# flynn-nrg/izpi

Measured on AMD Instinct MI355X. Metric: Msamples/sec (pixels x spp) at 1024x1024/512spp, higher is better.
Workload: dtype f64

## Files before the change

include/izpi_gpu.h:

```cpp
#ifndef IZPI_GPU_H
#define IZPI_GPU_H
#include <stddef.h>
#include <stdint.h>
#include "izpi_types.h"

#ifdef __cplusplus
extern "C" {
#endif

typedef struct izpi_ctx izpi_ctx;

typedef struct izpi_scene_desc {
  uint32_t abi_version;
  uint32_t num_nodes;
  uint32_t num_prims;
  uint32_t num_tris, num_spheres, num_lights, num_materials, num_textures;
  uint32_t num_spd;
  uint32_t flags;
  uint64_t num_texels;
  const izpi_bvh4_node* nodes;
  const uint32_t* prim_ref;
  const double* tri_v0;
  const double* tri_v1;
  const double* tri_v2;
  const double* tri_e1;
  const double* tri_e2;
  const double* tri_normal;
  const double* tri_tangent;
  const double* tri_bitangent;
  const double* tri_uv;
  const double* tri_area;
  const uint32_t* tri_mat;
  const double* sph_center0;
  const double* sph_center1;
  const double* sph_time;
  const double* sph_radius;
  const uint32_t* sph_mat;
  const uint32_t* light_ref;
  const izpi_material* materials;
  const izpi_texture* textures;
  const double* texels;
  const double* spd_wavelengths;
  const double* spd_values;
  izpi_camera camera;
} izpi_scene_desc;

enum {
  IZPI_SCENE_QUANTIZED_BVH = 1
};

enum {
  IZPI_SAMPLER_NORMAL = 1,
  IZPI_SAMPLER_COLOUR = 2,
  IZPI_SAMPLER_WIREFRAME = 3,
  IZPI_SAMPLER_ALBEDO = 4,
  IZPI_SAMPLER_SPECTRAL = 5
};
enum {
  IZPI_OUT_CANVAS = 0,
  IZPI_OUT_PACKED = 1
};

typedef struct izpi_render_tuning {
  uint32_t slots;
  uint32_t chunk_units;
  uint32_t rec_dense;
  uint32_t pool_div;
  uint32_t trace_chunk;
  uint32_t refill_min;
  uint32_t prim_weight;
  uint32_t flags;
  uint64_t tail_paths;
  uint32_t peer_timeout_ms;
  uint32_t pad_tuning;
} izpi_render_tuning;
enum {
  IZPI_TUNE_NO_DIST = 1,
  IZPI_TUNE_GENERAL_TRACE = 2,
  IZPI_TUNE_NO_LEAF_SHORTCUT = 4,
  IZPI_TUNE_SCALAR_SLAB = 8,
  IZPI_TUNE_NO_TAIL = 16,
  IZPI_TUNE_PASS_LOG = 32,
  IZPI_TUNE_NO_LDS_BVH = 64,
  IZPI_TUNE_NO_RAY_LDS = 128,
  IZPI_TUNE_NO_PRIM_LDS = 256,
  IZPI_TUNE_NO_PLACE_PICK = 512,
  IZPI_TUNE_NO_QNODES = 1024,
  IZPI_TUNE_NO_SHADE_STAGE = 2048
};

typedef struct izpi_render_req {
  uint32_t width, height;
  uint32_t spp;
  uint32_t max_depth;
  uint32_t sampler;
  uint32_t out_layout;
  uint32_t num_tiles;
  uint32_t num_bg_spd;
  const uint32_t* tiles;
  const double* bg_spd_wavelengths;
  const double* bg_spd_values;
  double background[3];
  uint64_t seed;
  uint32_t post;
  uint32_t abi_version;
  double exposure;
  const izpi_render_tuning* tuning;
  uint32_t accumulation;
  uint32_t pad_req;
  double ink[3];
} izpi_render_req;

enum { IZPI_ACC_RECURSIVE = 0, IZPI_ACC_FORWARD = 1 };

enum { IZPI_POST_NONE = 0, IZPI_POST_SPECTRAL = 1,
       IZPI_POST_GAMMA_CLAMP = 2 };

enum { IZPI_FILTER_GAMMA = 1,
       IZPI_FILTER_CLAMP = 2   };
#define IZPI_MAX_FILTERS 8

typedef struct izpi_render_stats {
  uint64_t rays;
  uint64_t node_visits;
  uint64_t tri_tests;
  uint64_t sph_tests;
  uint64_t light_tri_tests;
  uint64_t light_sph_tests;
  uint64_t samples;
  double kernel_ms;
  double shade_ms;
  double total_ms;
  uint32_t launches;
  uint32_t pad;
  uint64_t node_steps, prim_steps, leaf_shortcuts;
  double tail_ms;
  uint64_t tail_node_visits, tail_tri_tests, tail_sph_tests;
  uint64_t parks;
  uint64_t workspace_bytes, scene_bytes;
  uint32_t slots, rec_dense, pool_blocks, chunk_spp;
  double alloc_ms;
} izpi_render_stats;

typedef struct izpi_hit {
  double t, u, v;
  double p[3];
  double normal[3];
  uint32_t prim_ref;
  uint32_t hit;
} izpi_hit;

int izpi_gpu_open(int device, izpi_ctx** out);
int izpi_gpu_close(izpi_ctx* ctx);
const char* izpi_gpu_last_error(izpi_ctx* ctx);

int izpi_gpu_upload_scene(izpi_ctx* ctx, const izpi_scene_desc* scene);

int izpi_gpu_render(izpi_ctx* ctx, const izpi_render_req* req, double* out_host, izpi_render_stats* stats);

int izpi_gpu_prepare(izpi_ctx* ctx, const izpi_render_req* req);

int izpi_gpu_render_device(izpi_ctx* ctx, const izpi_render_req* req, double* out_dev, izpi_render_stats* stats);

int izpi_gpu_unpack_tiles(izpi_ctx* ctx, const izpi_render_req* req, const double* packed_dev, double* canvas_dev);

int izpi_gpu_spectral_post(izpi_ctx* ctx, const double* xyz_dev, double* rgba_dev, uint32_t width, uint32_t height,
                           double exposure);

int izpi_gpu_postprocess(izpi_ctx* ctx, double* canvas_dev, uint32_t width, uint32_t height, const uint32_t* filters,
                         const double* params, uint32_t num_filters);

typedef struct izpi_denoise_params {
  uint32_t iterations;
  uint32_t flags;
  double sigma_colour, sigma_normal, sigma_albedo;
} izpi_denoise_params;
#define IZPI_DENOISE_MAX_ITERATIONS 8
#define IZPI_DENOISE_DEFAULT_ITERATIONS 5
#define IZPI_DENOISE_DEFAULT_SIGMA_COLOUR 1.0
#define IZPI_DENOISE_DEFAULT_SIGMA_NORMAL 0.5
#define IZPI_DENOISE_DEFAULT_SIGMA_ALBEDO 0.5
int izpi_gpu_denoise_device(izpi_ctx* ctx, const double* colour_dev, const double* normal_dev, const double* albedo_dev,
                            double* out_dev, uint32_t width, uint32_t height, const izpi_denoise_params* p,
                            double* device_ms);
int izpi_gpu_denoise(izpi_ctx* ctx, const double* colour, const double* normal, const double* albedo, double* out,
                     uint32_t width, uint32_t height, const izpi_denoise_params* p, double* device_ms);

enum { IZPI_BVH_LBVH = 0,
       IZPI_BVH_PLOC = 1,
       IZPI_BVH_SAH = 0x100 };
int izpi_gpu_build_bvh4(izpi_ctx* ctx, const double* boxes, uint32_t n, uint32_t leaf_max, uint32_t method,
                        izpi_bvh4_node* nodes, uint32_t max_nodes, uint32_t* num_nodes, uint32_t* order, double* build_ms);

typedef struct izpi_multi izpi_multi;
int izpi_gpu_multi_open(const int* devices, uint32_t num_devices, izpi_multi** out);
int izpi_gpu_multi_close(izpi_multi* m);
const char* izpi_gpu_multi_last_error(izpi_multi* m);
uint32_t izpi_gpu_multi_size(izpi_multi* m);
izpi_ctx* izpi_gpu_multi_context(izpi_multi* m, uint32_t i);
int izpi_gpu_multi_upload_scene(izpi_multi* m, const izpi_scene_desc* scene);
int izpi_gpu_multi_prepare(izpi_multi* m, const izpi_render_req* req);
int izpi_gpu_multi_render(izpi_multi* m, const izpi_render_req* req, double* out_host, izpi_render_stats* stats);

#define IZPI_COMM_ID_BYTES 128
int izpi_gpu_comm_id(uint8_t* id );
int izpi_gpu_comm_init(izpi_ctx* ctx, uint32_t nranks, uint32_t rank, const uint8_t* id );
int izpi_gpu_render_rank(izpi_ctx* ctx, const izpi_render_req* req, double* out_dev, izpi_render_stats* stats);

int izpi_gpu_progress(izpi_ctx* ctx, uint64_t* samples_done, uint64_t* samples_total);
int izpi_gpu_multi_progress(izpi_multi* m, uint64_t* samples_done, uint64_t* samples_total);

enum { IZPI_SNAP_CANVAS = 0, IZPI_SNAP_DISPLAY = 1 };
int izpi_gpu_progressive_begin(izpi_ctx* ctx, const izpi_render_req* req, uint32_t step_spp);
int izpi_gpu_progressive_step(izpi_ctx* ctx, uint32_t spp, izpi_render_stats* stats);
int izpi_gpu_progressive_snapshot(izpi_ctx* ctx, uint32_t form, double* out_host);
int izpi_gpu_progressive_snapshot_device(izpi_ctx* ctx, uint32_t form, double* out_dev);
int izpi_gpu_progressive_end(izpi_ctx* ctx);
int izpi_gpu_multi_progressive_begin(izpi_multi* m, const izpi_render_req* req, uint32_t step_spp);
int izpi_gpu_multi_progressive_step(izpi_multi* m, uint32_t spp, izpi_render_stats* stats);
int izpi_gpu_multi_progressive_snapshot(izpi_multi* m, uint32_t form, double* out_host);
int izpi_gpu_multi_progressive_end(izpi_multi* m);

enum { IZPI_PROG_NOISE = 1 };
enum { IZPI_SNAP_NOISE = 2 };
typedef struct izpi_noise_params {
  double threshold, floor, tolerated;
  uint32_t min_spp;
  uint32_t flags;
} izpi_noise_params;
#define IZPI_NOISE_DEFAULT_THRESHOLD 0.25
#define IZPI_NOISE_DEFAULT_FLOOR 0.01
#define IZPI_NOISE_DEFAULT_TOLERATED 0.05
#define IZPI_NOISE_DEFAULT_MIN_SPP 8
typedef struct izpi_noise_stats {
  uint64_t pixels, nonfinite, above;
  double max_error, sum_error, device_ms;
  uint32_t done, converged;
} izpi_noise_stats;
int izpi_gpu_progressive_begin_ex(izpi_ctx* ctx, const izpi_render_req* req, uint32_t step_spp, uint32_t flags);
int izpi_gpu_progressive_noise(izpi_ctx* ctx, const izpi_noise_params* p, izpi_noise_stats* out);
int izpi_gpu_progressive_converge(izpi_ctx* ctx, const izpi_noise_params* p, izpi_render_stats* stats,
// ... 17 lines not shown
```

izpi_amd/_native.py:

```python
import ctypes as C
from pathlib import Path

ROOT = Path(__file__).resolve().parents[1]
LIB_PATH = ROOT / "izpi_amd" / "_lib" / "libizpi_gpu.so"

c_double_p = C.POINTER(C.c_double)
c_uint32_p = C.POINTER(C.c_uint32)
c_float_p = C.POINTER(C.c_float)

COMM_ID_BYTES = 128
IZPI_OK, IZPI_ERR_INVALID, IZPI_ERR_HIP, IZPI_ERR_NO_SCENE, IZPI_ERR_UNSUPPORTED, IZPI_ERR_DEVICE, IZPI_ERR_PEER = range(7)
IZPI_ABI_VERSION = 4
ACC_RECURSIVE, ACC_FORWARD = 0, 1
SCENE_QUANTIZED_BVH = 1
PRIM_TRIANGLE, PRIM_SPHERE = 0, 1
TEX_CONSTANT, TEX_IMAGE, TEX_SPECTRAL_GAUSSIAN, TEX_SPECTRAL_TABULATED, TEX_SPECTRAL_IMAGE = 1, 3, 5, 7, 9
MAT_DIELECTRIC, MAT_DIFFUSE_LIGHT, MAT_ISOTROPIC, MAT_LAMBERT, MAT_METAL, MAT_PBR = 1, 2, 3, 4, 5, 6
MATF_BEER_LAMBERT = 1
SAMPLER_NORMAL, SAMPLER_COLOUR, SAMPLER_WIREFRAME, SAMPLER_ALBEDO, SAMPLER_SPECTRAL = 1, 2, 3, 4, 5
OUT_CANVAS, OUT_PACKED = 0, 1
POST_NONE, POST_SPECTRAL, POST_GAMMA_CLAMP = 0, 1, 2
SNAP_CANVAS, SNAP_DISPLAY, SNAP_NOISE = 0, 1, 2
PROG_NOISE = 1
NOISE_DEFAULT_THRESHOLD, NOISE_DEFAULT_FLOOR, NOISE_DEFAULT_TOLERATED, NOISE_DEFAULT_MIN_SPP = 0.25, 0.01, 0.05, 8
FILTER_GAMMA, FILTER_CLAMP = 1, 2
MAX_FILTERS = 8
HOST_SKIP_BVH = 1
BVH_LBVH, BVH_PLOC = 0, 1
BVH_SAH = 0x100
BVH_PLOC_SAH = BVH_PLOC | BVH_SAH
DISPLACE_PER_TRIANGLE, DISPLACE_MESH = 0, 1
DISPLACE_MAX_LEVELS = 16
DENOISE_MAX_ITERATIONS = 8
DENOISE_DEFAULT_ITERATIONS = 5
DENOISE_DEFAULT_SIGMA_COLOUR, DENOISE_DEFAULT_SIGMA_NORMAL, DENOISE_DEFAULT_SIGMA_ALBEDO = 1.0, 0.5, 0.5


def prim_ref(kind, idx):
    return (kind << 31) | idx


class BVH4Node(C.Structure):
    _fields_ = [("min_x", C.c_float * 4), ("min_y", C.c_float * 4), ("min_z", C.c_float * 4),
                ("max_x", C.c_float * 4), ("max_y", C.c_float * 4), ("max_z", C.c_float * 4),
                ("child", C.c_int32 * 4), ("prim_count", C.c_int32 * 4)]


class Texture(C.Structure):
    _fields_ = [("kind", C.c_uint32), ("width", C.c_uint32), ("height", C.c_uint32),
                ("spd_offset", C.c_uint32), ("spd_count", C.c_uint32), ("pad0", C.c_uint32),
                ("texel_offset", C.c_uint64), ("value", C.c_double * 3),
                ("peak", C.c_double), ("center", C.c_double), ("width_nm", C.c_double)]


class Material(C.Structure):
    _fields_ = [("kind", C.c_uint32), ("albedo_tex", C.c_int32), ("spectral_tex", C.c_int32),
                ("normal_tex", C.c_int32), ("roughness_tex", C.c_int32), ("metalness_tex", C.c_int32),
                ("absorb_tex", C.c_int32), ("flags", C.c_uint32), ("ref_idx", C.c_double),
                ("fuzz", C.c_double), ("rgb", C.c_double * 3), ("pad1", C.c_double)]


class Camera(C.Structure):
    _fields_ = [("origin", C.c_double * 3), ("lower_left", C.c_double * 3), ("horizontal", C.c_double * 3),
                ("vertical", C.c_double * 3), ("u", C.c_double * 3), ("v", C.c_double * 3),
                ("lens_radius", C.c_double), ("time0", C.c_double), ("time1", C.c_double), ("exposure", C.c_double)]


class SceneDesc(C.Structure):
    _fields_ = [("abi_version", C.c_uint32), ("num_nodes", C.c_uint32), ("num_prims", C.c_uint32),
                ("num_tris", C.c_uint32), ("num_spheres", C.c_uint32), ("num_lights", C.c_uint32),
                ("num_materials", C.c_uint32), ("num_textures", C.c_uint32), ("num_spd", C.c_uint32),
                ("flags", C.c_uint32), ("num_texels", C.c_uint64),
                ("nodes", C.POINTER(BVH4Node)), ("prim_ref", c_uint32_p),
                ("tri_v0", c_double_p), ("tri_v1", c_double_p), ("tri_v2", c_double_p),
                ("tri_e1", c_double_p), ("tri_e2", c_double_p), ("tri_normal", c_double_p),
                ("tri_tangent", c_double_p), ("tri_bitangent", c_double_p), ("tri_uv", c_double_p),
                ("tri_area", c_double_p), ("tri_mat", c_uint32_p),
                ("sph_center0", c_double_p), ("sph_center1", c_double_p), ("sph_time", c_double_p),
                ("sph_radius", c_double_p), ("sph_mat", c_uint32_p),
                ("light_ref", c_uint32_p), ("materials", C.POINTER(Material)), ("textures", C.POINTER(Texture)),
                ("texels", c_double_p), ("spd_wavelengths", c_double_p), ("spd_values", c_double_p),
                ("camera", Camera)]


class RenderTuning(C.Structure):
    _fields_ = [("slots", C.c_uint32), ("chunk_units", C.c_uint32), ("rec_dense", C.c_uint32),
                ("pool_div", C.c_uint32), ("trace_chunk", C.c_uint32), ("refill_min", C.c_uint32),
                ("prim_weight", C.c_uint32), ("flags", C.c_uint32), ("tail_paths", C.c_uint64),
                ("peer_timeout_ms", C.c_uint32), ("pad_tuning", C.c_uint32)]


TUNE_NO_DIST, TUNE_GENERAL_TRACE, TUNE_NO_LEAF_SHORTCUT, TUNE_SCALAR_SLAB, TUNE_NO_TAIL, TUNE_PASS_LOG = 1, 2, 4, 8, 16, 32
TUNE_NO_LDS_BVH = 64
TUNE_NO_RAY_LDS = 128
TUNE_NO_PRIM_LDS = 256
TUNE_NO_QNODES = 1024
TUNE_NO_SHADE_STAGE = 2048


def tuning(**kw):
    t = RenderTuning()
    for k, v in kw.items():
        if k == "flags" and not isinstance(v, int):
            v = sum(v)
        setattr(t, k, v)
    return t


class RenderReq(C.Structure):
    _fields_ = [("width", C.c_uint32), ("height", C.c_uint32), ("spp", C.c_uint32), ("max_depth", C.c_uint32),
                ("sampler", C.c_uint32), ("out_layout", C.c_uint32), ("num_tiles", C.c_uint32),
                ("num_bg_spd", C.c_uint32), ("tiles", c_uint32_p), ("bg_spd_wavelengths", c_double_p),
                ("bg_spd_values", c_double_p), ("background", C.c_double * 3), ("seed", C.c_uint64),
                ("post", C.c_uint32), ("abi_version", C.c_uint32), ("exposure", C.c_double),
                ("tuning", C.POINTER(RenderTuning)), ("accumulation", C.c_uint32), ("pad_req", C.c_uint32),
                ("ink", C.c_double * 3)]


class RenderStats(C.Structure):
    _fields_ = [("rays", C.c_uint64), ("node_visits", C.c_uint64), ("tri_tests", C.c_uint64),
                ("sph_tests", C.c_uint64), ("light_tri_tests", C.c_uint64), ("light_sph_tests", C.c_uint64),
                ("samples", C.c_uint64), ("kernel_ms", C.c_double), ("shade_ms", C.c_double),
                ("total_ms", C.c_double), ("launches", C.c_uint32), ("pad", C.c_uint32),
                ("node_steps", C.c_uint64), ("prim_steps", C.c_uint64), ("leaf_shortcuts", C.c_uint64),
                ("tail_ms", C.c_double), ("tail_node_visits", C.c_uint64), ("tail_tri_tests", C.c_uint64),
                ("tail_sph_tests", C.c_uint64), ("parks", C.c_uint64), ("workspace_bytes", C.c_uint64),
                ("scene_bytes", C.c_uint64), ("slots", C.c_uint32), ("rec_dense", C.c_uint32),
                ("pool_blocks", C.c_uint32), ("chunk_spp", C.c_uint32), ("alloc_ms", C.c_double)]

    def as_dict(self):
        return {k: getattr(self, k) for k, _ in self._fields_ if k != "pad"}


class DenoiseParams(C.Structure):
    _fields_ = [("iterations", C.c_uint32), ("flags", C.c_uint32), ("sigma_colour", C.c_double),
                ("sigma_normal", C.c_double), ("sigma_albedo", C.c_double)]


def denoise_params(iterations=DENOISE_DEFAULT_ITERATIONS, sigma_colour=DENOISE_DEFAULT_SIGMA_COLOUR,
                   sigma_normal=DENOISE_DEFAULT_SIGMA_NORMAL, sigma_albedo=DENOISE_DEFAULT_SIGMA_ALBEDO):
    return DenoiseParams(int(iterations), 0, float(sigma_colour), float(sigma_normal), float(sigma_albedo))


class NoiseParams(C.Structure):
    _fields_ = [("threshold", C.c_double), ("floor", C.c_double), ("tolerated", C.c_double),
                ("min_spp", C.c_uint32), ("flags", C.c_uint32)]


def noise_params(threshold=NOISE_DEFAULT_THRESHOLD, floor=NOISE_DEFAULT_FLOOR, tolerated=NOISE_DEFAULT_TOLERATED,
                 min_spp=NOISE_DEFAULT_MIN_SPP):
    return NoiseParams(float(threshold), float(floor), float(tolerated), int(min_spp), 0)


class NoiseStats(C.Structure):
    _fields_ = [("pixels", C.c_uint64), ("nonfinite", C.c_uint64), ("above", C.c_uint64),
                ("max_error", C.c_double), ("sum_error", C.c_double), ("device_ms", C.c_double),
                ("done", C.c_uint32), ("converged", C.c_uint32)]

    def as_dict(self):
        return {k: getattr(self, k) for k, _ in self._fields_}


class Hit(C.Structure):
    _fields_ = [("t", C.c_double), ("u", C.c_double), ("v", C.c_double), ("p", C.c_double * 3),
                ("normal", C.c_double * 3), ("prim_ref", C.c_uint32), ("hit", C.c_uint32)]


class TriIn(C.Structure):
    _fields_ = [("v0", C.c_double * 3), ("v1", C.c_double * 3), ("v2", C.c_double * 3),
                ("uv", C.c_double * 6), ("material", C.c_uint32), ("pad", C.c_uint32)]


class SphereIn(C.Structure):
    _fields_ = [("center", C.c_double * 3), ("radius", C.c_double), ("material", C.c_uint32), ("pad", C.c_uint32)]


class CameraIn(C.Structure):
    _fields_ = [("look_from", C.c_double * 3), ("look_at", C.c_double * 3), ("vup", C.c_double * 3),
                ("vfov", C.c_double), ("aspect", C.c_double), ("aperture", C.c_double), ("focus_dist", C.c_double),
                ("time0", C.c_double), ("time1", C.c_double), ("exposure", C.c_double)]


class SceneInput(C.Structure):
    _fields_ = [("num_tris", C.c_uint32), ("num_spheres", C.c_uint32), ("num_materials", C.c_uint32),
                ("num_textures", C.c_uint32), ("num_spd", C.c_uint32), ("pad0", C.c_uint32),
                ("num_texels", C.c_uint64), ("tris", C.c_void_p), ("spheres", C.c_void_p),
                ("materials", C.POINTER(Material)), ("textures", C.POINTER(Texture)), ("texels", c_double_p),
                ("spd_wavelengths", c_double_p), ("spd_values", c_double_p), ("camera", CameraIn),
                ("aspect_override", C.c_double), ("bvh_seed", C.c_uint64)]


COLOUR_RGB, COLOUR_SPECTRAL = 1, 2
OBJ_IGNORE_NORMALS, OBJ_IGNORE_MATERIALS, OBJ_IGNORE_TEXTURES = 1, 2, 4
OBJ_FACE_POLYGON = 1


class ProtoInfo(C.Structure):
    _fields_ = [("colour_representation", C.c_uint32), ("stream_triangles", C.c_uint32),
                ("total_triangles", C.c_uint64), ("num_triangles", C.c_uint32), ("num_streamed_triangles", C.c_uint32),
                ("num_spheres", C.c_uint32), ("num_materials", C.c_uint32), ("num_image_textures", C.c_uint32),
                ("num_displacement_maps", C.c_uint32), ("num_background", C.c_uint32), ("pad", C.c_uint32),
                ("name", C.c_char_p), ("version", C.c_char_p), ("warnings", C.c_char_p)]


class ObjInfo(C.Structure):
    _fields_ = [("has_normals", C.c_uint32), ("has_uv", C.c_uint32), ("ignore_materials", C.c_uint32),
                ("ignore_normals", C.c_uint32), ("ignore_textures", C.c_uint32), ("num_groups", C.c_uint32),
                ("num_materials", C.c_uint32), ("pad", C.c_uint32), ("num_vertices", C.c_uint64),
                ("num_normals", C.c_uint64), ("num_uvs", C.c_uint64), ("centre", C.c_double * 3),
                ("object_name", C.c_char_p)]


class ObjGroup(C.Structure):
    _fields_ = [("name", C.c_char_p), ("material", C.c_char_p), ("face_type", C.c_uint32), ("is_null", C.c_uint32),
                ("num_faces", C.c_uint64), ("num_face_vertices", C.c_uint64)]


class ObjMaterial(C.Structure):
    _fields_ = [("name", C.c_char_p), ("kd", C.c_double * 3), ("ka", C.c_double * 3), ("ks", C.c_double * 3),
                ("num_kd", C.c_uint32), ("num_ka", C.c_uint32), ("num_ks", C.c_uint32), ("pad", C.c_uint32),
                ("ns", C.c_double), ("ni", C.c_double), ("d", C.c_double), ("sharpness", C.c_int64),
                ("illum", C.c_int64)]


ABI_STRUCTS = [BVH4Node, Texture, Material, Camera, SceneDesc, RenderReq, RenderStats, Hit, TriIn, SphereIn, CameraIn,
               SceneInput, ProtoInfo, ObjInfo, ObjGroup, ObjMaterial, RenderTuning, DenoiseParams, NoiseParams, NoiseStats]

EXPORTS = [
    "izpi_gpu_open", "izpi_gpu_close", "izpi_gpu_prepare", "izpi_gpu_multi_prepare", "izpi_gpu_last_error", "izpi_gpu_upload_scene", "izpi_gpu_render",
    "izpi_gpu_render_device", "izpi_gpu_unpack_tiles", "izpi_gpu_output_bytes", "izpi_gpu_trace",
    "izpi_gpu_ray_aabb4", "izpi_gpu_gomath", "izpi_gpu_spectral_post", "izpi_gpu_postprocess",
    "izpi_gpu_build_bvh4", "izpi_gpu_multi_open", "izpi_gpu_multi_close", "izpi_gpu_multi_last_error",
    "izpi_gpu_multi_size", "izpi_gpu_multi_context", "izpi_gpu_multi_upload_scene", "izpi_gpu_multi_render",
    "izpi_gpu_comm_id", "izpi_gpu_comm_init", "izpi_gpu_render_rank", "izpi_gpu_debug_fault", "izpi_gpu_debug_realloc", "izpi_gpu_progress", "izpi_gpu_multi_progress", "izpi_host_build_scene_ex", "izpi_host_scene_prim_boxes", "izpi_host_scene_set_bvh", "izpi_host_scene_set_flags",
    "izpi_host_build_scene", "izpi_host_scene_desc", "izpi_host_scene_stack_bound", "izpi_host_scene_build_ms",
    "izpi_host_scene_free", "izpi_host_last_error", "izpi_host_tiles", "izpi_host_share_units", "izpi_host_share_tiles", "izpi_host_share_block", "izpi_host_assemble_shares", "izpi_host_bvh_leaf_max", "izpi_host_gomath", "izpi_abi_struct_size",
    "izpi_scene_parse_text", "izpi_scene_parse_binary", "izpi_scene_serialize", "izpi_scene_info", "izpi_scene_image_file",
    "izpi_scene_set_image", "izpi_scene_add_triangles", "izpi_scene_background", "izpi_scene_to_input",
    "izpi_scene_material_name", "izpi_scene_free", "izpi_light_source", "izpi_light_source_name",
    "izpi_obj_parse", "izpi_obj_info_get", "izpi_obj_copy_vertices", "izpi_obj_group_get", "izpi_obj_copy_faces",
    "izpi_obj_material_get", "izpi_obj_translate", "izpi_obj_scale", "izpi_obj_rotate",
    "izpi_obj_group_to_triangles", "izpi_obj_free",
    "izpi_gpu_displace", "izpi_host_displace", "izpi_scene_displacement_file", "izpi_scene_set_displacement_map",
    "izpi_scene_set_displacer",
    "izpi_gpu_progressive_begin", "izpi_gpu_progressive_step", "izpi_gpu_progressive_snapshot",
    "izpi_gpu_progressive_snapshot_device", "izpi_gpu_progressive_end",
    "izpi_gpu_multi_progressive_begin", "izpi_gpu_multi_progressive_step", "izpi_gpu_multi_progressive_snapshot",
    "izpi_gpu_multi_progressive_end",
    "izpi_gpu_denoise_device", "izpi_gpu_denoise", "izpi_host_denoise",
    "izpi_gpu_progressive_begin_ex", "izpi_gpu_progressive_noise", "izpi_gpu_progressive_converge",
# ... 144 lines not shown
```

izpi_amd/csrc/izpi_dev.h:

```cpp
#pragma once
#include <hip/hip_runtime.h>
#include <stdint.h>
#include "../../include/izpi_gpu.h"
#include "gomath.h"
#include "scene_records.h"

#define IZPI_DEV __device__ __forceinline__

namespace izd {

struct DevScene {
  const GInner* inner;
  const GInnerQ* innerq;
  const GLeaf* leaves;
  const GPrim* prims;
  const GShade* shade;
  const GTriTex* tritex;
  const GLight* lights;
  const izpi_material* materials;
  const izpi_texture* textures;
  const double4* mat_const;
  const MatTex* mat_tex;
  const double* texels;
  const double* spd_wl;
  const double* spd_val;
  int32_t root;
  uint32_t num_lights;
  uint32_t nan_free_bounds;
  uint32_t leaf_shortcut;
  uint32_t tri_only;
  uint32_t no_pathlen;
  uint32_t num_inner;
  uint32_t num_prims;
  izpi_camera cam;
  uint32_t lds_bytes;
  uint32_t time_free;
  uint32_t quantized;
#ifdef IZPI_SHADOW
  const GInner* sh_inner;
  const GLeaf* sh_leaves;
  const GPrim* sh_prims;
#endif
};

struct RenderParams {
  uint32_t width, height, spp, max_depth;
  uint32_t chunk_spp;
  uint32_t s0;
  uint32_t num_pixels;
  uint32_t tile_w, tile_h;
  uint32_t total_units;
  uint32_t lanes;
  uint32_t num_bg_spd;
  const uint32_t* tiles;
  const double* bg_wl;
  const double* bg_val;
  double background[3];
  uint64_t seed;
  double* out;
  double* recs;
  uint32_t* head;
  unsigned long long* counters;
  uint32_t* error;
};

struct Lcg {
  uint32_t s;
  IZPI_DEV double next() {
    s = 1664525u * s + 1013904223u;
    return (double)s / 4294967296.0;
  }
};
IZPI_DEV uint64_t splitmix64(uint64_t x) {
  uint64_t z = x + 0x9E3779B97F4A7C15ull;
  z = (z ^ (z >> 30)) * 0xBF58476D1CE4E5B9ull;
  z = (z ^ (z >> 27)) * 0x94D049BB133111EBull;
  return z ^ (z >> 31);
}
#define IZPI_CAMERA_STREAM_SALT 0xD6E8FEB86659FD93ull

IZPI_DEV int64_t go_int(double x) {
  if (x != x || x >= 9223372036854775808.0 || x < -9223372036854775808.0) return INT64_MIN;
  return (int64_t)x;
}

struct V3 { double x, y, z; };
IZPI_DEV V3 mk(double x, double y, double z) { V3 r; r.x = x; r.y = y; r.z = z; return r; }
IZPI_DEV V3 ld3(const double* p) { return mk(p[0], p[1], p[2]); }
IZPI_DEV V3 add(V3 a, V3 b) { return mk(a.x + b.x, a.y + b.y, a.z + b.z); }
IZPI_DEV V3 sub(V3 a, V3 b) { return mk(a.x - b.x, a.y - b.y, a.z - b.z); }
IZPI_DEV V3 mul(V3 a, V3 b) { return mk(a.x * b.x, a.y * b.y, a.z * b.z); }
IZPI_DEV V3 smul(V3 a, double t) { return mk(a.x * t, a.y * t, a.z * t); }
IZPI_DEV bool sdiv_plain(double x) {
  return ((uint32_t)(__double2hiint(x) >> 20) & 0x7FFu) - (1023u - 300u) <= 600u;
}
IZPI_DEV V3 sdiv(V3 a, double t) {
  const int px = (int)sdiv_plain(a.x) | (int)(a.x == 0.0), py = (int)sdiv_plain(a.y) | (int)(a.y == 0.0),
            pz = (int)sdiv_plain(a.z) | (int)(a.z == 0.0);
  const bool plain = ((int)sdiv_plain(t) & px & py & pz) != 0;
  if (plain) {
    double r = __builtin_amdgcn_rcp(t);
    double e = __builtin_fma(-t, r, 1.0);
    r = __builtin_fma(r, e, r);
    e = __builtin_fma(-t, r, 1.0);
    r = __builtin_fma(r, e, r);
    auto q1 = [&](double n) {
      const double q = n * r;
      const double res = __builtin_fma(-t, q, n);
      return __builtin_amdgcn_div_fixup(__builtin_amdgcn_div_fmas(res, r, q, false), t, n);
    };
    return mk(q1(a.x), q1(a.y), q1(a.z));
  }
  return mk(a.x / t, a.y / t, a.z / t);
}
IZPI_DEV double dot(V3 a, V3 b) { return (a.x * b.x) + (a.y * b.y) + (a.z * b.z); }
IZPI_DEV V3 cross(V3 a, V3 b) { return mk((a.y * b.z) - (a.z * b.y), -((a.x * b.z) - (a.z * b.x)), (a.x * b.y) - (a.y * b.x)); }
IZPI_DEV double sqlen(V3 a) { return (a.x * a.x) + (a.y * a.y) + (a.z * a.z); }
IZPI_DEV double length(V3 a) { return gm::sqrt(sqlen(a)); }
IZPI_DEV V3 unit(V3 a) { return sdiv(a, length(a)); }
IZPI_DEV V3 lerp(V3 a, V3 b, double t) {
  return mk((1 - t) * a.x + t * b.x, (1 - t) * a.y + t * b.y, (1 - t) * a.z + t * b.z);
}
IZPI_DEV bool bad(double x) { return x != x || gm::is_inf(x, 0); }
IZPI_DEV V3 denan(V3 v) { return mk(bad(v.x) ? 0.0 : v.x, bad(v.y) ? 0.0 : v.y, bad(v.z) ? 0.0 : v.z); }

struct Onb {
  V3 u, v, w;
  IZPI_DEV void build(V3 n) {
    w = unit(n);
    V3 a = gm::abs(w.x) > 0.9 ? mk(0, 1, 0) : mk(1, 0, 0);
    v = unit(cross(w, a));
    u = cross(w, v);
  }
  IZPI_DEV V3 local(V3 a) const { return add(add(smul(u, a.x), smul(v, a.y)), smul(w, a.z)); }
};

IZPI_DEV V3 random_cosine_direction(Lcg& r) {
  double r1 = r.next();
  double r2 = r.next();
  double z = gm::sqrt(1 - r2);
  double phi = 6.283185307179586 * r1;
  double sp, cp;
  gm::sincos_nonneg(phi, &sp, &cp);
  double x = cp * 2 * gm::sqrt(r2);
  double y = sp * 2 * gm::sqrt(r2);
  return mk(x, y, z);
}
IZPI_DEV V3 random_to_sphere(double radius, double dist2, Lcg& r) {
  double r1 = r.next();
  double r2 = r.next();
  double z = 1 + r2 * (gm::sqrt(1 - radius * radius / dist2) - 1);
  double phi = 6.283185307179586 * r1;
  double sp, cp;
  gm::sincos_nonneg(phi, &sp, &cp);
  double x = cp * gm::sqrt(1 - z * z);
  double y = sp * gm::sqrt(1 - z * z);
  return mk(x, y, z);
}
IZPI_DEV V3 random_in_unit_sphere(Lcg& r) {
  for (;;) {
    double x = r.next(), y = r.next(), z = r.next();
    V3 p = sub(smul(mk(x, y, z), 2.0), mk(1.0, 1.0, 1.0));
    if (sqlen(p) < 1.0) return p;
  }
}

IZPI_DEV float max32(float a, float b) { return a > b ? a : b; }
IZPI_DEV float min32(float a, float b) { return a < b ? a : b; }
IZPI_DEV bool slab(float mnx, float mny, float mnz, float mxx, float mxy, float mxz, float ox, float oy, float oz,
                   float ix, float iy, float iz, float tmax) {
  float t0x = (mnx - ox) * ix, t1x = (mxx - ox) * ix;
  if (t0x > t1x) { float t = t0x; t0x = t1x; t1x = t; }
  float t0y = (mny - oy) * iy, t1y = (mxy - oy) * iy;
  if (t0y > t1y) { float t = t0y; t0y = t1y; t1y = t; }
  float t0z = (mnz - oz) * iz, t1z = (mxz - oz) * iz;
  if (t0z > t1z) { float t = t0z; t0z = t1z; t1z = t; }
  float tn = max32(max32(t0x, t0y), t0z);
  float tf = min32(min32(t1x, t1y), t1z);
  return tn <= tf && tf >= 0 && tn <= tmax;
}

typedef float f32x2 __attribute__((ext_vector_type(2)));
IZPI_DEV void slab4_fast(float4 mnx, float4 mny, float4 mnz, float4 mxx, float4 mxy, float4 mxz, float ox, float oy,
                         float oz, float ix, float iy, float iz, float tmax, uint64_t (&h)[4]) {
  const f32x2 o_x = {ox, ox}, o_y = {oy, oy}, o_z = {oz, oz};
  const f32x2 i_x = {ix, ix}, i_y = {iy, iy}, i_z = {iz, iz};
  const f32x2 a0x = (f32x2{mnx.x, mnx.y} - o_x) * i_x, a1x = (f32x2{mnx.z, mnx.w} - o_x) * i_x;
  const f32x2 b0x = (f32x2{mxx.x, mxx.y} - o_x) * i_x, b1x = (f32x2{mxx.z, mxx.w} - o_x) * i_x;
  const f32x2 a0y = (f32x2{mny.x, mny.y} - o_y) * i_y, a1y = (f32x2{mny.z, mny.w} - o_y) * i_y;
  const f32x2 b0y = (f32x2{mxy.x, mxy.y} - o_y) * i_y, b1y = (f32x2{mxy.z, mxy.w} - o_y) * i_y;
// ... 87 lines not shown
```

izpi_amd/csrc/izpi_gpu.hip:

```cpp
#include "izpi_kern.h"
#include "noise.h"
#include "scene_pack.h"

#include <array>

using izpi_internal::Double4;
using izpi_internal::pack_scene;
using izpi_internal::PackedScene;
using izpi_internal::PlanCache;
using izpi_internal::PlanInput;
using izpi_internal::SideLayout;
using izpi_internal::WorkspacePlan;

__global__ void __launch_bounds__(256) k_spectral_post(const double* in, double* out, uint32_t W, uint32_t H,
                                                       double exposure) {
  __shared__ double ys[18][18];
  const int tx = threadIdx.x & 15, ty = threadIdx.x >> 4;
  const int x0 = blockIdx.x * 16, y0 = blockIdx.y * 16;
  for (int i = threadIdx.x; i < 18 * 18; i += 256) {
    const int hx = x0 + (i % 18) - 1, hy = y0 + (i / 18) - 1;
    ys[i / 18][i % 18] = (hx >= 0 && hx < (int)W && hy >= 0 && hy < (int)H) ? in[((size_t)hy * W + hx) * 4 + 1] : 0.0;
  }
  __syncthreads();
  const int x = x0 + tx, y = y0 + ty;
  if (x >= (int)W || y >= (int)H) return;
  const size_t pi = ((size_t)y * W + x) * 4;
  const double2 xy = *reinterpret_cast<const double2*>(in + pi), za = *reinterpret_cast<const double2*>(in + pi + 2);
  double X = xy.x, Y = xy.y, Z = za.x;
  const double cur = ys[ty + 1][tx + 1];
  if (cur > 0) {
    double nb[8];
    int nn = 0;
    for (int dy = -1; dy <= 1; dy++)
      for (int dx = -1; dx <= 1; dx++) {
        if (dx == 0 && dy == 0) continue;
        const int nx = x + dx, ny = y + dy;
        if (nx >= 0 && nx < (int)W && ny >= 0 && ny < (int)H) {
          const double v = ys[ty + 1 + dy][tx + 1 + dx];
          if (v > 0) nb[nn++] = v;
        }
      }
    if (nn >= 3) {
      double sum = 0.0;
      for (int i = 0; i < nn; i++) sum += nb[i];
      const double mean = sum / (double)nn;
      double vs = 0.0;
      for (int i = 0; i < nn; i++) { const double d = nb[i] - mean; vs += d * d; }
      const double stddev = gm::sqrt(vs / (double)nn);
      const double threshold = mean + 2.5 * stddev;
      if (cur > threshold && threshold > 0) {
        const double ratio = threshold / cur;
        X *= ratio; Y *= ratio; Z *= ratio;
      }
    }
  }
  X *= exposure; Y *= exposure; Z *= exposure;
  double2 rg, ba;
  rg.x = 1.6410234 * X + -0.3248033 * Y + -0.2364247 * Z;
  rg.y = -0.6636629 * X + 1.6153316 * Y + 0.0167563 * Z;
  ba.x = 0.0117219 * X + -0.0082845 * Y + 0.9883949 * Z;
  ba.y = za.y;
  *reinterpret_cast<double2*>(out + pi) = rg;
  *reinterpret_cast<double2*>(out + pi + 2) = ba;
}

struct PostFilters {
  uint32_t n;
  uint32_t kind[IZPI_MAX_FILTERS];
  double param[IZPI_MAX_FILTERS];
};

__global__ void __launch_bounds__(256) k_postprocess(double* canvas, uint64_t num_pixels, const PostFilters pf) {
  const uint64_t i = (uint64_t)blockIdx.x * 256 + threadIdx.x;
  if (i >= num_pixels) return;
  double2* p = reinterpret_cast<double2*>(canvas + i * 4);
  double2 rg = p[0], ba = p[1];
  double c[3] = {rg.x, rg.y, ba.x};
  for (uint32_t f = 0; f < pf.n; f++) {
    if (pf.kind[f] == IZPI_FILTER_GAMMA) {
      for (int k = 0; k < 3; k++) c[k] = gm::sqrt(c[k]);
    } else {
      const double mx = pf.param[f];
      for (int k = 0; k < 3; k++) c[k] = c[k] < mx ? c[k] : mx;
    }
  }
  p[0] = make_double2(c[0], c[1]);
  p[1] = make_double2(c[2], ba.y);
}

__host__ __device__ inline bool packed_target(const uint32_t* tiles, uint32_t p, uint32_t tile_w, uint32_t tile_h,
                                              uint32_t height, uint32_t* x, uint32_t* row) {
  const uint32_t tile_px = tile_w * tile_h;
  const uint32_t tile = p / tile_px, in_tile = p % tile_px;
  *x = tiles[4 * tile] + in_tile % tile_w;
  *row = height - (tiles[4 * tile + 1] + in_tile / tile_w);
  return *row < height;
}
__global__ void k_unpack(const uint32_t* tiles, uint32_t num_pixels, uint32_t tile_w, uint32_t tile_h, uint32_t width,
                         uint32_t height, const double* packed, double* canvas) {
  const uint32_t p = blockIdx.x * 256 + threadIdx.x;
  if (p >= num_pixels) return;
  uint32_t x, row;
  if (packed_target(tiles, p, tile_w, tile_h, height, &x, &row)) {
    const double* s = packed + (size_t)p * 4;
    double* o = canvas + ((size_t)row * width + x) * 4;
    o[0] = s[0]; o[1] = s[1]; o[2] = s[2]; o[3] = s[3];
  }
}

__global__ void __launch_bounds__(256) k_cpart_reduce(const unsigned long long* cpart, uint32_t rows,
                                                      unsigned long long* counters) {
  __shared__ unsigned long long red[256];
  unsigned long long v = 0;
  for (uint32_t r = threadIdx.x; r < rows; r += 256) v += cpart[(size_t)r * CNT_N + blockIdx.x];
  red[threadIdx.x] = v;
  __syncthreads();
  for (uint32_t h = 128; h > 0; h >>= 1) {
    if (threadIdx.x < h) red[threadIdx.x] += red[threadIdx.x + h];
    __syncthreads();
  }
  if (threadIdx.x == 0) counters[blockIdx.x] += red[0];
}

__global__ void k_trace_setup(const double* rays, uint32_t n, RayOD* ray, uint32_t* kind, double2* tminmax, uint32_t* qn) {
  const uint32_t i = blockIdx.x * 256 + threadIdx.x;
  if (i == 0) *qn = n;
  if (i >= n) return;
  const double* r = rays + (size_t)i * 8;
  RayOD h;
  for (int k = 0; k < 3; k++) { h.o[k] = r[k]; h.d[k] = r[3 + k]; }
  ray[i] = h;
  kind[i] = RAY_PATHLEN;
  tminmax[i] = make_double2(r[6], r[7]);
}
__global__ void k_trace_records(const DevScene sc, const RayOD* rr, const double2* hit, uint32_t n, izpi_hit* out) {
  const uint32_t i = blockIdx.x * 256 + threadIdx.x;
  if (i >= n) return;
  izpi_hit h;
  memset(&h, 0, sizeof(h));
  h.prim_ref = 0xFFFFFFFFu;
  HitOut c;
  const double2* rec = hit + 2 * (size_t)i;
  c.t = rec[0].x; c.prim = hit_prim(rec[0]); c.u = rec[1].x; c.v = rec[1].y; c.pad = 0;
  if (c.prim >= 0) {
    const RayOD R = rr[i];
    HitRec hr;
    const GShade gs = sc.shade[c.prim];
    hit_record(sc, c, rec + 1, gs, mk(R.o[0], R.o[1], R.o[2]), mk(R.d[0], R.d[1], R.d[2]), 0.0, true, hr);
    const GPrim& p = sc.prims[c.prim];
    h.hit = 1; h.t = hr.t; h.u = hr.u; h.v = hr.v;
    h.p[0] = hr.p.x; h.p[1] = hr.p.y; h.p[2] = hr.p.z;
    h.normal[0] = hr.n.x; h.normal[1] = hr.n.y; h.normal[2] = hr.n.z;
    h.prim_ref = IZPI_PRIM_REF(p.kind, p.index);
  }
  out[i] = h;
}

__global__ void k_aabb4(const float* boxes, const float* rays, uint32_t n, uint8_t* masks) {
  const uint32_t i = blockIdx.x * 256 + threadIdx.x;
  if (i >= n) return;
  const float* b = boxes + (size_t)i * 24;
// ... 278 lines not shown

int allocate(izpi_ctx* ctx, const izpi_render_req* req, const RequestShape& rs, const WorkspacePlan& plan, const Tracer& tr,
             const RenderCall& call) {
  const auto bufs = ctx_buffers(ctx);
  const size_t bytes[RENDER_BUFS] = {plan.samples_bytes, plan.recs_bytes, plan.pool_bytes, plan.ring_bytes,
                                     plan.running_bytes, plan.state_bytes, tr.spill_bytes};
  int rc = IZPI_OK;
  if (rs.preview) {
    if ((rc = session_keeps_sums(ctx, call, ctx->running_cap < plan.running_bytes))) return rc;
    for (size_t k = 0; k < RENDER_BUFS && !rc; k++) rc = grow(ctx, bufs[k].p, bufs[k].cap, bytes[k]);
  } else {
    bool fresh = false;
    rc = grow_render_buffers(ctx, bufs.data(), bytes, &fresh);
    if (!rc && (rc = session_keeps_sums(ctx, call, fresh))) return rc;
  }
  if (!rc) rc = grow(ctx, (void**)&ctx->d_tiles, &ctx->tiles_cap, rs.tiles.size() * sizeof(uint32_t));
  if (!rc && !rs.preview) {
    if (req->num_bg_spd && (!req->bg_spd_wavelengths || !req->bg_spd_values)) { ctx->err = "num_bg_spd without the SPD arrays"; return IZPI_ERR_INVALID; }
    rc = grow(ctx, (void**)&ctx->d_bg, &ctx->bg_cap, (2 * (size_t)req->num_bg_spd + 1) * sizeof(double));
  }
  if (!rc) rc = grow(ctx, (void**)&ctx->d_cpart, &ctx->cpart_cap, (size_t)cpart_rows(ctx) * CNT_N * sizeof(unsigned long long));
  if (!rc && !rs.preview && !rs.fwd) rc = grow(ctx, (void**)&ctx->d_finq, &ctx->finq_cap, (size_t)ctx->num_cus * CPART_BLOCKS_PER_CU * FINQ_WORDS * FINQ_CAP * sizeof(unsigned long long));
  if (rc) ctx->plans[rs.preview].valid = false;
  return rc;
}

int touch_workspace(izpi_ctx* ctx, const WorkspacePlan& plan, const RenderCall& call, double alloc_ms) {
  hipStream_t st = ctx->stream;
  HIP_TRY(hipMemsetAsync(ctx->d_state, 0, plan.state_bytes, st));
  HIP_TRY(hipMemsetAsync(ctx->d_samples, 0, plan.samples_bytes, st));
  if (plan.recs_bytes) HIP_TRY(hipMemsetAsync(ctx->d_recs, 0, plan.recs_bytes, st));
  if (call.range.keep) {
    HIP_TRY(hipMemsetAsync(ctx->d_running, 0, plan.running_bytes, st));
    HIP_TRY(hipMemsetAsync(ctx->d_counters, 0, CNT_N * sizeof(unsigned long long), st));
  }
  HIP_TRY(hipStreamSynchronize(st));
  ctx->last = izpi_render_stats{};
  ctx->last.workspace_bytes = workspace_bytes(ctx);
  ctx->last.slots = plan.slots; ctx->last.chunk_spp = plan.chunk; ctx->last.alloc_ms = alloc_ms;
  return IZPI_OK;
}

int begin_frame(izpi_ctx* ctx, const izpi_render_req* req, const RequestShape& rs, const WorkspacePlan& plan, const RenderCall& call,
                size_t nbg) {
  hipStream_t st = ctx->stream;
  HIP_TRY(hipMemcpyAsync(ctx->d_tiles, rs.tiles.data(), rs.tiles.size() * sizeof(uint32_t), hipMemcpyHostToDevice, st));
  if (nbg) {
    HIP_TRY(hipMemcpyAsync(ctx->d_bg, req->bg_spd_wavelengths, nbg * sizeof(double), hipMemcpyHostToDevice, st));
    HIP_TRY(hipMemcpyAsync(ctx->d_bg + nbg, req->bg_spd_values, nbg * sizeof(double), hipMemcpyHostToDevice, st));
  }
  if (!call.range.keep) {
    HIP_TRY(hipMemsetAsync(ctx->d_running, 0, plan.running_bytes, st));
    HIP_TRY(hipMemsetAsync(ctx->d_counters, 0, CNT_N * sizeof(unsigned long long), st));
  }
  HIP_TRY(hipMemsetAsync(ctx->d_cpart, 0, (size_t)cpart_rows(ctx) * CNT_N * sizeof(unsigned long long), st));
  HIP_TRY(hipMemsetAsync(ctx->d_misc, 0, 8 * MISC_STRIDE * sizeof(uint32_t), st));
  return IZPI_OK;
}

ShadeParams shade_params(izpi_ctx* ctx, const izpi_render_req* req, const RequestShape& rs, const WorkspacePlan& plan) {
  ShadeParams sp{};
  sp.width = req->width; sp.height = req->height; sp.tile_w = rs.tw; sp.tile_h = rs.th; sp.slots = plan.slots;
  sp.max_depth = rs.preview ? 1 : req->max_depth;
  sp.tiles = ctx->d_tiles; sp.seed = req->seed; sp.out = ctx->d_samples;
  sp.background[0] = req->background[0]; sp.background[1] = req->background[1]; sp.background[2] = req->background[2];
  sp.counters = ctx->d_counters; sp.cpart = ctx->d_cpart; sp.error = misc(ctx, 1);
  return sp;
}
void path_shade_params(izpi_ctx* ctx, const izpi_render_req* req, const DevScene& sc, const RequestShape& rs,
                       const WorkspacePlan& plan, size_t nbg, ShadeParams& sp) {
  sp.num_bg_spd = (uint32_t)nbg;
  sp.bg_sorted = nbg >= 2;
  for (size_t i = 1; i < nbg; i++)
    if (!(req->bg_spd_wavelengths[i - 1] <= req->bg_spd_wavelengths[i])) sp.bg_sorted = 0;
  sp.bg_wl = ctx->d_bg; sp.bg_val = ctx->d_bg + nbg;
  sp.rec_dense = plan.rec_dense; sp.rec_pool = plan.rec_pool; sp.pool_shift = plan.pool_shift;
  sp.recs = rs.fwd ? nullptr : ctx->d_recs; sp.mat_const = sc.mat_const; sp.head = misc(ctx, 0);
  sp.num_mc = ctx->num_materials; sp.num_tex = ctx->num_textures; sp.num_spd = ctx->num_spd;
  sp.pool = plan.rec_pool ? ctx->d_pool : nullptr; sp.pool_ring = plan.rec_pool ? ctx->d_ring : nullptr;
  sp.pool_ctr = plan.rec_pool ? ctx->d_pool_ctr : nullptr;
  sp.finq = ctx->d_finq;
}
void stage_tables(const izpi_ctx* ctx, const izpi_render_req* req, const izpi_render_tuning& tu, const RequestShape& rs,
                  const WorkspacePlan& plan, size_t nbg, DevScene& sc, ShadeParams& sp) {
  sp.staged = ctx->num_materials <= MC_LDS && ctx->num_materials <= MAT_LDS && sc.num_lights <= LT_LDS &&
              ctx->num_textures <= TEX_LDS && ctx->num_spd <= SPD_LDS && nbg <= BG_LDS;
  sp.prims_staged = sc.num_prims <= PR_LDS && !(tu.flags & IZPI_TUNE_NO_PRIM_LDS);
  if (sp.staged && (req->sampler == IZPI_SAMPLER_SPECTRAL || ctx->num_spd)) sp.staged = 2;
  if (rs.fwd && req->sampler == IZPI_SAMPLER_COLOUR && ctx->matset == 0 && sp.staged == 1 && !plan.rec_pool && !plan.time &&
      !plan.cold && !(tu.flags & IZPI_TUNE_NO_SHADE_STAGE))
    sp.prims_staged = 0;
  sc.lds_bytes = sp.prims_staged ? lds_off::END : sp.staged == 2 ? lds_off::SPECTRAL_END : sp.staged ? lds_off::COLOUR_END : 0;
  if (tu.flags & IZPI_TUNE_PASS_LOG)
    fprintf(stderr, "IZPI_SHADE_TABLES tables=%u prims=%u lds_bytes=%u\n", sp.staged, sp.prims_staged, sc.lds_bytes);
}
WaveParams wave_params(izpi_ctx* ctx, const WorkspacePlan& plan, const ShadeParams& sp) {
  WaveParams wp{};
  wp.in = bind_side(ctx->d_state, plan, plan.side[0]); wp.out = bind_side(ctx->d_state, plan, plan.side[1]);
  wp.trace_next = misc(ctx, 2); wp.slots = plan.slots;
  wp.read_kind = !ctx->sc.no_pathlen ? 1u : 0u;
  wp.hit_uv = plan.uv ? 1u : 0u;
  wp.pool_ctr = sp.pool_ctr;
  wp.cpart = ctx->d_cpart;
  return wp;
}
PreviewParams preview_params(izpi_ctx* ctx, const izpi_render_req* req, const WorkspacePlan& plan) {
  PreviewParams pp{};
  pp.buf = bind_side(ctx->d_state, plan, plan.side[0]);
  pp.tminmax = plan.tminmax ? (double2*)(ctx->d_state + plan.side[0].tminmax) : nullptr;
  pp.slots = plan.slots;
  pp.verts = ctx->d_triverts;
  if (req->abi_version >= 4)
    for (int k = 0; k < 3; k++) pp.ink[k] = req->ink[k];
  return pp;
}
AccumParams accum_params(izpi_ctx* ctx, const izpi_render_req* req, const RequestShape& rs, double* out_dev) {
  AccumParams ap{};
  ap.num_pixels = rs.num_pixels; ap.spp = req->spp; ap.width = req->width; ap.height = req->height;
  ap.tile_w = rs.tw; ap.tile_h = rs.th; ap.out_layout = req->out_layout;
  ap.sampler = rs.preview ? (uint32_t)IZPI_SAMPLER_COLOUR : req->sampler;
  ap.tiles = ctx->d_tiles; ap.samples = ctx->d_samples; ap.running = ctx->d_running; ap.out = out_dev;
  return ap;
}

int guard_status(izpi_ctx* ctx, uint32_t guard) {
  if (!guard) return IZPI_OK;
  ctx->err = guard & 1u   ? "device guard: traversal stack overflow"
             : guard & 2u ? "device guard: unknown material kind"
                            : "device guard: no overflow record block in k_tail";
  return IZPI_ERR_DEVICE;
}

int render_body(izpi_ctx* ctx, const izpi_render_req* req, const RenderCall& call, double* out_dev) {
  const auto t_body0 = std::chrono::steady_clock::now();
  auto host_ms = [&t_body0]() { return std::chrono::duration<double, std::milli>(std::chrono::steady_clock::now() - t_body0).count(); };
  RequestShape rs;
  int rc = check_request(ctx, req, &rs);
  if (rc) return rc;
  const SampleRange& sr = call.range;
  const uint32_t num_pixels = rs.num_pixels;
  if (sr.keep) {
    izpi_ctx::Session& ss = ctx->session;
    ss.run_tiles = rs.tiles; ss.tile_w = rs.tw; ss.tile_h = rs.th; ss.num_pixels = num_pixels;
  }
  const izpi_render_tuning& tu = tuning_of(req);
  const bool pass_log = (tu.flags & IZPI_TUNE_PASS_LOG) != 0;
  DevScene sc = ctx->sc;
  if (tu.flags & IZPI_TUNE_NO_LEAF_SHORTCUT) sc.leaf_shortcut = 0;
  if (tu.flags & IZPI_TUNE_SCALAR_SLAB) sc.nan_free_bounds = 0;
  Tracer tr;
  const double t_tiles = host_ms();
  if ((rc = make_tracer(ctx, tu, !ctx->sc.tri_only || ctx->any_uv, &tr))) return rc;
  if (pass_log)
    fprintf(stderr, "IZPI_TRACE_INSTANCE dist=%d tri=%d lds_bvh=%d ray_lds=%d q=%d\n", (int)tr.p2, (int)tr.tri, (int)tr.lds_bvh,
            (int)tr.ray_lds, (int)tr.qnodes);
  const double t_tracer = host_ms();
  PlanCache& cache = ctx->plans[rs.preview];
  PlanInput in = plan_input(ctx, req, rs, tu, call.size_spp);
  const bool reuse = cache.find(in) != nullptr;
  if (!reuse) in.avail = available_bytes(ctx);
  const double t_meminfo = host_ms();
  if (!reuse) cache.store(in, plan_workspace(in));
  const WorkspacePlan& plan = cache.plan;
  const double t_sized = host_ms();
  const auto t_alloc0 = std::chrono::steady_clock::now();
  if ((rc = allocate(ctx, req, rs, plan, tr, call))) return rc;
  const double alloc_ms = std::chrono::duration<double, std::milli>(std::chrono::steady_clock::now() - t_alloc0).count();
  if (call.prepare_only) return touch_workspace(ctx, plan, call, alloc_ms);
  hipStream_t st = ctx->stream;
  if (pass_log) HIP_TRY(hipEventRecord(ctx->evb[0], st));
  const size_t nbg = rs.preview ? 0 : req->num_bg_spd;
  if ((rc = begin_frame(ctx, req, rs, plan, call, nbg))) return rc;
  ShadeParams sp = shade_params(ctx, req, rs, plan);
  AccumParams ap = accum_params(ctx, req, rs, out_dev);
  if (!rs.preview) {
    path_shade_params(ctx, req, sc, rs, plan, nbg, sp);
    stage_tables(ctx, req, tu, rs, plan, nbg, sc, sp);
  }

  const RunInput run{num_pixels, plan.chunk, plan.pool_blocks, sr};
  RunTimes times;
  float total_ms = 0;
  const double t_launch = host_ms();
  HIP_TRY(hipEventRecord(ctx->ev0, st));
  if (pass_log) {
    HIP_TRY(hipEventSynchronize(ctx->ev0));
    float prep = 0;
    HIP_TRY(hipEventElapsedTime(&prep, ctx->evb[0], ctx->ev0));
    fprintf(stderr, "IZPI_T ev0_synced %.3f prep_gpu_ms %.3f body_start %.3f\n", diag_clock_ms(), prep,
            diag_clock_ms() - host_ms());
  }
  if (rs.preview) {
    const PreviewParams pp = preview_params(ctx, req, plan);
    rc = run_preview(ctx, req, sc, tr, sp, pp, ap, run, &times);
  } else {
    WaveParams wp = wave_params(ctx, plan, sp);
    const ShadeKernels* k = ctx->kernels[req->sampler == IZPI_SAMPLER_SPECTRAL][rs.fwd];
    if (!k || (!rs.fwd && k->rec_doubles != plan.D)) {
      ctx->err = "the shading instance and the workspace plan disagree on the record stride";
      return IZPI_ERR_INVALID;
    }
    rc = run_wavefront(ctx, req, sc, tr, *k, sp, wp, ap, run, &times);
  }
  if (rc) return rc;
  hipLaunchKernelGGL(k_cpart_reduce, dim3(CNT_N), dim3(256), 0, st, ctx->d_cpart, cpart_rows(ctx), ctx->d_counters);
  HIP_TRY(hipGetLastError());
  HIP_TRY(hipEventRecord(ctx->ev1, st));
  if (!sr.keep && (rc = apply_post(ctx, req, out_dev))) return rc;
  const double t_issued = host_ms();
  HIP_TRY(hipEventSynchronize(ctx->ev1));
  if (pass_log)
    fprintf(stderr, "IZPI_HOST tiles %.3f tracer %.3f meminfo %.3f sized %.3f allocated %.3f launched %.3f issued %.3f done %.3f ms\n",
            t_tiles, t_tracer, t_meminfo, t_sized, t_sized + alloc_ms, t_launch, t_issued, host_ms());
  HIP_TRY(hipEventElapsedTime(&total_ms, ctx->ev0, ctx->ev1));
  unsigned long long cnt[CNT_N];
  uint32_t guard = 0;
  HIP_TRY(hipMemcpy(cnt, ctx->d_counters, sizeof(cnt), hipMemcpyDeviceToHost));
  HIP_TRY(hipMemcpy(&guard, misc(ctx, 1), sizeof(guard), hipMemcpyDeviceToHost));
  izpi_render_stats& s = ctx->last;
  memset(&s, 0, sizeof(s));
  s.rays = cnt[CNT_RAYS]; s.node_visits = cnt[CNT_NODES]; s.tri_tests = cnt[CNT_TRI]; s.sph_tests = cnt[CNT_SPH];
  s.light_tri_tests = cnt[CNT_LTRI]; s.light_sph_tests = cnt[CNT_LSPH];
  s.samples = (uint64_t)num_pixels * sr.end;
  s.kernel_ms = times.trace_ms; s.shade_ms = times.shade_ms; s.total_ms = total_ms; s.launches = times.launches; s.tail_ms = times.tail_ms;
  s.node_steps = cnt[CNT_NSTEP]; s.prim_steps = cnt[CNT_PSTEP]; s.leaf_shortcuts = cnt[CNT_SHORT];
  s.tail_node_visits = cnt[CNT_TAIL_NODES]; s.tail_tri_tests = cnt[CNT_TAIL_TRI]; s.tail_sph_tests = cnt[CNT_TAIL_SPH];
  s.parks = cnt[CNT_PARK];
  s.workspace_bytes = workspace_bytes(ctx);
  s.scene_bytes = ctx->scene_bytes;
  s.slots = plan.slots; s.rec_dense = rs.fwd ? 0 : plan.rec_dense; s.pool_blocks = plan.pool_blocks; s.chunk_spp = plan.chunk;
  s.alloc_ms = alloc_ms;
  if (!sr.keep && plan.rec_pool && s.parks * 64 > s.rays && plan.pool_blocks < plan.slots) ctx->pool_grow++;
#ifdef IZPI_SHADE_CLOCKS
  fprintf(stderr, "IZPI_SHADE_CLOCKS item %llu refill %llu push %llu mat %llu finish %llu mix %llu lpdf %llu entry %llu tex %llu "
          "res_barrier1 %llu res_atomics %llu res_barrier2 %llu (wave cycles; res_atomics: thread 0 only)\n",
          cnt[CNT_SCLK_ITEM], cnt[CNT_SCLK_REFILL], cnt[CNT_SCLK_PUSH], cnt[CNT_SCLK_MAT], cnt[CNT_SCLK_FIN],
          cnt[CNT_SCLK_MIX], cnt[CNT_SCLK_LPDF], cnt[CNT_SCLK_ENTRY], cnt[CNT_SCLK_TEX], cnt[CNT_SCLK_RB1],
          cnt[CNT_SCLK_RATOM], cnt[CNT_SCLK_RB2]);
#endif
#ifdef IZPI_SHADOW
  fprintf(stderr, "IZPI_SHADOW spill_stores %llu spill_loads %llu (entries)\n", cnt[CNT_CLK_REFILL], cnt[CNT_CLK_NODE]);
#endif
#ifdef IZPI_TRACE_CLOCKS
  fprintf(stderr, "IZPI_TRACE_CLOCKS refill %llu node %llu prim %llu advance %llu (wave cycles)\n", cnt[CNT_CLK_REFILL],
          cnt[CNT_CLK_NODE], cnt[CNT_CLK_PRIM], cnt[CNT_CLK_ADV]);
#endif
  return guard_status(ctx, guard);
}

int render_impl(izpi_ctx* ctx, const izpi_render_req* req, const RenderCall& call, double* out_dev) {
  if (session_open(ctx)) return IZPI_ERR_INVALID;
  ctx->prog_done.store(0, std::memory_order_relaxed);
  ctx->prog_total.store(0, std::memory_order_relaxed);
  const int rc = render_body(ctx, req, call, out_dev);
  ctx->prog_done.store(ctx->prog_total.load(std::memory_order_relaxed), std::memory_order_relaxed);
  return rc;
}

struct Shares {
  std::vector<uint32_t> all;
  uint32_t n = 1;
  uint32_t tw = 0, th = 0;
  size_t block = 0;
  std::vector<uint32_t> mine(uint32_t r) const {
    std::vector<uint32_t> t(all.size());
    t.resize(4 * (size_t)izpi_host_share_tiles(all.data(), (uint32_t)(all.size() / 4), r, n, t.data()));
    return t;
  }
};

size_t share_block(size_t ntiles, uint32_t tw, uint32_t th, uint32_t n) { return ((ntiles + n - 1) / n) * (size_t)tw * th * 4; }

int make_shares(izpi_ctx* ctx, const izpi_render_req* req, uint32_t n, Shares& sh) {
  if (!req || req->width == 0 || req->height == 0) { ctx->err = "invalid render request"; return IZPI_ERR_INVALID; }
  if (req->out_layout != IZPI_OUT_CANVAS) { ctx->err = "multi-GPU renders produce a canvas (IZPI_OUT_CANVAS)"; return IZPI_ERR_INVALID; }
  std::vector<uint32_t> tiles;
  int rc = request_tiles(ctx, req, tiles);
  if (rc) return rc;
  sh.all.resize(4 * tiles.size());
  sh.all.resize(4 * (size_t)izpi_host_share_units(tiles.data(), (uint32_t)(tiles.size() / 4), n, sh.all.data()));
  if (!validate_tiles(req, sh.all.data(), (uint32_t)(sh.all.size() / 4), &sh.tw, &sh.th)) {
    ctx->err = "tiles must be non-empty, in bounds and equal-sized";
    return IZPI_ERR_INVALID;
  }
  sh.n = n;
  sh.block = share_block(sh.all.size() / 4, sh.tw, sh.th, n);
  return IZPI_OK;
}

int share_buffers(izpi_ctx* ctx, const Shares& sh, bool root, size_t canvas_bytes = 0) {
  int rc = grow(ctx, (void**)&ctx->d_share, &ctx->share_cap, sh.block * sizeof(double));
  if (!rc && root) rc = grow(ctx, (void**)&ctx->d_gather, &ctx->gather_cap, (size_t)sh.n * sh.block * sizeof(double));
  if (!rc && root && canvas_bytes) rc = grow(ctx, (void**)&ctx->d_out, &ctx->out_cap, canvas_bytes);
  return rc;
}

int render_share(izpi_ctx* ctx, const izpi_render_req* req, const Shares& sh, uint32_t r, bool prepare_only = false) {
  const std::vector<uint32_t> mine = sh.mine(r);
  memset(&ctx->last, 0, sizeof(ctx->last));
  if (mine.empty()) return IZPI_OK;
  izpi_render_req q = request_copy(req);
  q.num_tiles = (uint32_t)(mine.size() / 4);
  q.tiles = mine.data();
  q.out_layout = IZPI_OUT_PACKED;
  q.post = IZPI_POST_NONE;
  return render_impl(ctx, &q, one_shot(&q, prepare_only), prepare_only ? nullptr : ctx->d_share);
}

int assemble(izpi_ctx* ctx, const izpi_render_req* req, const Shares& sh, double* canvas_dev) {
  izpi_ctx* root = ctx;
  hipStream_t st = root->stream;
  for (uint32_t r = 0; r < sh.n; r++) {
    const std::vector<uint32_t> t = sh.mine(r);
    if (t.empty()) continue;
    int rc = grow(root, (void**)&root->d_utiles, &root->utiles_cap, sh.all.size() * sizeof(uint32_t));
    if (rc) return rc;
    HIP_TRY(hipMemcpyAsync(root->d_utiles, t.data(), t.size() * sizeof(uint32_t), hipMemcpyHostToDevice, st));
    const uint32_t np = (uint32_t)(t.size() / 4) * sh.tw * sh.th;
    hipLaunchKernelGGL(k_unpack, dim3((np + 255) / 256), dim3(256), 0, st, root->d_utiles, np, sh.tw, sh.th, req->width,
                       req->height, root->d_gather + (size_t)r * sh.block, canvas_dev);
    HIP_TRY(hipGetLastError());
    HIP_TRY(hipStreamSynchronize(st));
  }
  int rc = apply_post(root, req, canvas_dev);
  if (rc) return rc;
  HIP_TRY(hipStreamSynchronize(st));
  return IZPI_OK;
}

int session_copy_request(izpi_ctx::Session& ss, const izpi_render_req* req, std::string& err) {
  ss = izpi_ctx::Session{};
  ss.req = request_copy(req);
  ss.tuning = tuning_of(req);
  ss.req.tuning = req->tuning ? &ss.tuning : nullptr;
  if (ss.req.num_tiles) {
    if (!ss.req.tiles) { err = "num_tiles without tiles"; return IZPI_ERR_INVALID; }
    ss.tiles.assign(ss.req.tiles, ss.req.tiles + 4 * (size_t)ss.req.num_tiles);
    ss.req.tiles = ss.tiles.data();
  }
  if (ss.req.num_bg_spd) {
    if (!ss.req.bg_spd_wavelengths || !ss.req.bg_spd_values) { err = "num_bg_spd without the SPD arrays"; return IZPI_ERR_INVALID; }
    ss.bg_wl.assign(ss.req.bg_spd_wavelengths, ss.req.bg_spd_wavelengths + ss.req.num_bg_spd);
    ss.bg_val.assign(ss.req.bg_spd_values, ss.req.bg_spd_values + ss.req.num_bg_spd);
    ss.req.bg_spd_wavelengths = ss.bg_wl.data();
    ss.req.bg_spd_values = ss.bg_val.data();
  }
  return IZPI_OK;
}

void session_drop(izpi_ctx* ctx) {
  ctx->session = izpi_ctx::Session{};
  ctx->prog_done.store(0, std::memory_order_relaxed);
  ctx->prog_total.store(0, std::memory_order_relaxed);
}

int session_zero_moments(izpi_ctx* ctx) {
  izpi_ctx::Session& ss = ctx->session;
  const size_t bytes = (size_t)ss.num_pixels * 3 * sizeof(double);
  const int rc = grow(ctx, (void**)&ctx->d_moments, &ctx->moments_cap, bytes);
  if (rc) return rc;
  HIP_TRY(hipMemsetAsync(ctx->d_moments, 0, bytes, ctx->stream));
  HIP_TRY(hipStreamSynchronize(ctx->stream));
  ss.noise = true;
  return IZPI_OK;
}

int session_begin(izpi_ctx* ctx, const izpi_render_req* req, uint32_t step_spp, uint32_t flags = 0) {
  if (ctx->session.open) { ctx->err = "a progressive session is already open"; return IZPI_ERR_INVALID; }
  if (!req || step_spp == 0) { ctx->err = "progressive_begin: a request and step_spp >= 1"; return IZPI_ERR_INVALID; }
  if (flags & ~(uint32_t)IZPI_PROG_NOISE) { ctx->err = "progressive_begin: unknown flags"; return IZPI_ERR_INVALID; }
  izpi_ctx::Session& ss = ctx->session;
  int rc = session_copy_request(ss, req, ctx->err);
  if (!rc) {
    ss.step_spp = std::min(step_spp, std::max(1u, ss.req.spp));
    rc = render_body(ctx, &ss.req, RenderCall{SampleRange{0, 0, true}, ss.step_spp, true}, nullptr);
  }
  if (!rc && (flags & IZPI_PROG_NOISE)) rc = session_zero_moments(ctx);
  if (rc) {
    const std::string why = ctx->err;
    session_drop(ctx);
    ctx->err = why;
    return rc;
  }
  ss.cum = izpi_render_stats{};
  ss.open = true;
  ctx->prog_done.store(0, std::memory_order_relaxed);
  ctx->prog_total.store((uint64_t)ss.num_pixels * ss.req.spp, std::memory_order_relaxed);
  return IZPI_OK;
}

int session_usable(izpi_ctx* ctx) {
  if (!ctx->session.open) { ctx->err = "no progressive session is open"; return IZPI_ERR_INVALID; }
  if (ctx->session.broken) { ctx->err = "the session's last step failed: end it"; return IZPI_ERR_INVALID; }
  return IZPI_OK;
}
// ... 48 lines not shown
  int rc = session_usable(ctx);
  if (rc) return rc;
  const izpi_noise_params p = params ? *params : nz::defaults();
  if (const char* bad = nz::check_params(p)) { ctx->err = bad; return IZPI_ERR_INVALID; }
  if ((rc = session_has_noise(ctx))) return rc;
  const izpi_ctx::Session& ss = ctx->session;
  hipStream_t st = ctx->stream;
  if ((rc = session_tiles(ctx))) return rc;
  const size_t blocks = ((size_t)ss.num_pixels + nz::BLOCK - 1) / nz::BLOCK;
  if ((rc = grow(ctx, (void**)&ctx->d_noisepart, &ctx->noisepart_cap, 5 * blocks * sizeof(double)))) return rc;
  NoiseParams np = noise_params(ctx);
  np.threshold = p.threshold; np.floor = p.floor;
  np.block_sums = ctx->d_noisepart;
  np.block_counts = (unsigned long long*)(ctx->d_noisepart + blocks);
  HIP_TRY(hipEventRecord(ctx->ev0, st));
  launch_noise_stats(st, np);
  HIP_TRY(hipGetLastError());
  HIP_TRY(hipEventRecord(ctx->ev1, st));
  std::vector<double> part(5 * blocks);
  HIP_TRY(hipMemcpyAsync(part.data(), ctx->d_noisepart, part.size() * sizeof(double), hipMemcpyDeviceToHost, st));
  HIP_TRY(hipStreamSynchronize(st));
  float ms = 0;
  HIP_TRY(hipEventElapsedTime(&ms, ctx->ev0, ctx->ev1));
  izpi_noise_stats s{};
  unsigned long long max_bits = 0;
  for (size_t b = 0; b < blocks; b++) {
    unsigned long long cnt[4];
    memcpy(cnt, part.data() + blocks + 4 * b, sizeof(cnt));
    s.pixels += cnt[0]; s.nonfinite += cnt[1]; s.above += cnt[2];
    max_bits = std::max(max_bits, cnt[3]);
    s.sum_error = s.sum_error + part[b];
  }
  s.max_error = gm::from_bits(max_bits);
  s.device_ms = ms;
  s.done = ss.done;
  s.converged = nz::converged(s.pixels, s.nonfinite, s.above, s.done, p);
  if (out) *out = s;
  return IZPI_OK;
}

template <class Step, class Noise, class Done>
int converge_loop(const izpi_noise_params* params, uint32_t cap, Step step, Noise noise, Done done, izpi_noise_stats* out) {
  const izpi_noise_params p = params ? *params : nz::defaults();
  izpi_noise_stats last{};
  int rc = IZPI_OK;
  while (!rc && done() < cap) {
    if ((rc = step())) break;
    if (done() < std::max(2u, p.min_spp)) continue;
    if ((rc = noise(&p, &last))) break;
    if (last.converged) break;
  }
  if (out) *out = last;
  return rc;
}

int session_snapshot(izpi_ctx* ctx, uint32_t form, double* out_dev) {
  int rc = session_usable(ctx);
  if (rc) return rc;
  const izpi_ctx::Session& ss = ctx->session;
  if (form != IZPI_SNAP_CANVAS && form != IZPI_SNAP_DISPLAY && form != IZPI_SNAP_NOISE) { ctx->err = "unknown snapshot form"; return IZPI_ERR_INVALID; }
  if (ss.done == 0) { ctx->err = "snapshot before the session's first sample"; return IZPI_ERR_INVALID; }
  if (form == IZPI_SNAP_NOISE && (rc = session_has_noise(ctx))) return rc;
  if (!out_dev) { ctx->err = "null output"; return IZPI_ERR_INVALID; }
  hipStream_t st = ctx->stream;
  if ((rc = session_tiles(ctx))) return rc;
  if (form == IZPI_SNAP_NOISE) {
    NoiseParams np = noise_params(ctx);
    np.out = out_dev;
    launch_noise_resolve(st, np);
    HIP_TRY(hipGetLastError());
    HIP_TRY(hipStreamSynchronize(st));
    return IZPI_OK;
  }
  ResolveParams rp{};
  rp.num_pixels = ss.num_pixels; rp.done = ss.done; rp.width = ss.req.width; rp.height = ss.req.height;
  rp.tile_w = ss.tile_w; rp.tile_h = ss.tile_h; rp.sampler = ss.req.sampler; rp.out_layout = ss.req.out_layout;
  rp.form = form; rp.exposure = ss.req.exposure;
  rp.tiles = ctx->d_tiles; rp.running = ctx->d_running; rp.out = out_dev;
  launch_resolve(st, rp);
  HIP_TRY(hipGetLastError());
  if (form == IZPI_SNAP_CANVAS && (rc = apply_post(ctx, &ss.req, out_dev))) return rc;
  HIP_TRY(hipStreamSynchronize(st));
  return IZPI_OK;
}

}

struct izpi_multi {
  std::vector<izpi_ctx*> ctx;
  std::string err;
  bool prog_open = false;
  izpi_ctx::Session session;
  Shares shares;
};

namespace {
int multi_shares(izpi_multi* m, const izpi_render_req* req, Shares& sh) {
  izpi_ctx* root = m->ctx[0];
  int rc = make_shares(root, req, (uint32_t)m->ctx.size(), sh);
  if (!rc && hipSetDevice(root->device) != hipSuccess) { root->err = "hipSetDevice"; rc = IZPI_ERR_HIP; }
  if (!rc) rc = share_buffers(root, sh, true, (size_t)req->width * req->height * 4 * sizeof(double));
  if (rc) m->err = root->err;
  return rc;
}

template <class F>
int on_every_device(izpi_multi* m, F fn) {
  const uint32_t G = (uint32_t)m->ctx.size();
  std::vector<int> rcs(G, IZPI_OK);
  std::vector<std::thread> th;
  for (uint32_t i = 0; i < G; i++) {
    th.emplace_back([&, i]() {
      izpi_ctx* c = m->ctx[i];
      if (hipSetDevice(c->device) != hipSuccess) { c->err = "hipSetDevice"; rcs[i] = IZPI_ERR_HIP; return; }
      rcs[i] = fn(i, c);
    });
  }
  for (std::thread& t : th) t.join();
  for (uint32_t i = 0; i < G; i++)
    if (rcs[i]) { m->err = "device " + std::to_string(i) + ": " + m->ctx[i]->err; return rcs[i]; }
  return IZPI_OK;
}

bool multi_lacks_noise(izpi_multi* m) {
  if (!m->session.noise) { m->err = "noise: the session was begun without IZPI_PROG_NOISE"; return true; }
  if (m->session.done < 2) { m->err = "noise: needs at least 2 samples"; return true; }
  return false;
}

bool multi_session_open(izpi_multi* m) {
  if (!m->prog_open) return false;
  m->err = "a progressive session is open";
  return true;
}

static_assert(sizeof(Double4) == sizeof(double4), "PackedScene::mat_const uploads as DevScene::mat_const");

int begin_upload(izpi_ctx* ctx, const izpi_scene_desc* d) {
  if (!ctx || !d) return IZPI_ERR_INVALID;
  if (d->abi_version < 1 || d->abi_version > IZPI_ABI_VERSION) { ctx->err = "ABI version mismatch"; return IZPI_ERR_INVALID; }
  if (session_open(ctx)) return IZPI_ERR_INVALID;
  HIP_TRY(hipSetDevice(ctx->device));
  HIP_TRY(hipStreamSynchronize(ctx->stream));
  free_scene(ctx);
  return IZPI_OK;
}

int upload_packed(izpi_ctx* ctx, const izpi_scene_desc* d, const PackedScene& ps) {
  DevScene& sc = ctx->sc;
  memset(&sc, 0, sizeof(sc));
  GInner* di; GInnerQ* dq; GLeaf* dl; GPrim* dp; GShade* dsh; GTriVerts* dtv; GTriTex* dtt; GLight* dlt;
  izpi_material* dm; Double4* dmc; MatTex* dmt; izpi_texture* dtx;
  double *dtex, *dswl, *dsv;
  UP(ps.inner.data(), ps.inner.size(), &di);
  UP(ps.innerq.data(), ps.innerq.size(), &dq);
  UP(ps.leaves.data(), ps.leaves.size(), &dl);
  UP(ps.prims.data(), ps.prims.size(), &dp);
  UP(ps.shade.data(), ps.shade.size(), &dsh);
  UP(ps.triverts.data(), ps.triverts.size(), &dtv);
  UP(ps.tritex.data(), ps.tritex.size(), &dtt);
  UP(ps.lights.data(), ps.lights.size(), &dlt);
  UP(d->materials, d->num_materials, &dm);
  UP(ps.mat_const.data(), ps.mat_const.size(), &dmc);
  UP(ps.mat_tex.data(), ps.mat_tex.size(), &dmt);
  UP(ps.textures.data(), ps.textures.size(), &dtx);
  UP(ps.texels.data(), ps.texels.size(), &dtex);
  UP(d->spd_wavelengths, d->num_spd, &dswl);
  UP(d->spd_values, d->num_spd, &dsv);
#ifdef IZPI_SHADOW
  {
    GInner* si; GLeaf* sl; GPrim* sp;
    UP(ps.inner.data(), ps.inner.size(), &si);
    UP(ps.leaves.data(), ps.leaves.size(), &sl);
    UP(ps.prims.data(), ps.prims.size(), &sp);
    sc.sh_inner = si; sc.sh_leaves = sl; sc.sh_prims = sp;
  }
#endif
  sc.inner = di; sc.innerq = dq; sc.leaves = dl; sc.prims = dp; sc.shade = dsh; sc.tritex = dtt; sc.lights = dlt;
  sc.materials = dm; sc.mat_const = (const double4*)dmc; sc.mat_tex = dmt; sc.textures = dtx; sc.texels = dtex;
  sc.spd_wl = dswl; sc.spd_val = dsv;
  sc.root = ps.root; sc.num_inner = ps.num_inner; sc.num_prims = d->num_prims; sc.num_lights = d->num_lights;
  sc.quantized = ps.quantized; sc.leaf_shortcut = ps.leaf_shortcut; sc.nan_free_bounds = ps.nan_free_bounds;
  sc.tri_only = ps.tri_only; sc.time_free = ps.time_free; sc.no_pathlen = ps.no_pathlen;
  sc.cam = d->camera;
  ctx->d_triverts = dtv;
  ctx->mat_ok_rgb = ps.mat_ok_rgb; ctx->mat_ok_spectral = ps.mat_ok_spectral;
  ctx->basic_materials = ps.basic_materials; ctx->matset = ps.matset;
  ctx->const_albedo = ps.const_albedo; ctx->any_uv = ps.any_uv;
  ctx->pool_grow = 0;
  ctx->stack_needed = ps.stack_needed;
  ctx->num_prims = d->num_prims;
  ctx->num_textures = d->num_textures;
  ctx->num_materials = d->num_materials;
  ctx->num_spd = d->num_spd;
  ctx->have_scene = true;
  ctx->plans[0].valid = ctx->plans[1].valid = false;
  Tracer tr;
  int rc = make_tracer(ctx, kDefaultTuning, !ctx->sc.tri_only || ctx->any_uv, &tr);
  const bool const_basic = ctx->basic_materials && ctx->const_albedo;
  for (int s = 0; s < 2; s++)
    for (int f = 1; f >= 0; f--) {
      const uint32_t sampler = s ? IZPI_SAMPLER_SPECTRAL : IZPI_SAMPLER_COLOUR;
      const ShadeKernels*& k = ctx->kernels[s][f];
      k = (s ? ctx->mat_ok_spectral : ctx->mat_ok_rgb) ? shade_instance(ctx->matset, const_basic, sampler, f != 0) : nullptr;
      if (!rc && k) rc = prepare_wavefront(ctx, *k);
    }
  if (!rc) rc = prepare_preview(ctx);
  return rc;
}
}

extern "C" {

int izpi_gpu_open(int device, izpi_ctx** out) {
  if (!out) return IZPI_ERR_INVALID;
  *out = nullptr;
  int n = 0;
  hipError_t e = hipGetDeviceCount(&n);
  if (e != hipSuccess || n == 0 || device < 0 || device >= n) return IZPI_ERR_HIP;
  if (hipSetDevice(device) != hipSuccess) return IZPI_ERR_HIP;
  izpi_ctx* ctx = new izpi_ctx();
  ctx->device = device;
  hipDeviceProp_t prop;
  bool ok = hipGetDeviceProperties(&prop, device) == hipSuccess;
  ctx->num_cus = ok ? prop.multiProcessorCount : 0;
  ok = ok && hipStreamCreateWithFlags(&ctx->stream, hipStreamNonBlocking) == hipSuccess &&
       hipEventCreate(&ctx->ev0) == hipSuccess && hipEventCreate(&ctx->ev1) == hipSuccess &&
       hipEventCreate(&ctx->ev2) == hipSuccess && hipEventCreate(&ctx->ev3) == hipSuccess &&
       hipHostMalloc((void**)&ctx->h_count, 9 * MISC_STRIDE * sizeof(uint32_t), hipHostMallocDefault) == hipSuccess &&
       hipMalloc((void**)&ctx->d_misc, 8 * MISC_STRIDE * sizeof(uint32_t)) == hipSuccess &&
       hipMalloc((void**)&ctx->d_pool_ctr, POOL_SHARDS * POOL_CTR_STRIDE * sizeof(unsigned long long)) == hipSuccess &&
       hipMalloc((void**)&ctx->d_counters, CNT_N * sizeof(unsigned long long)) == hipSuccess;
  for (int i = 0; ok && i < 3 * IZPI_PASS_BATCH; i++) ok = hipEventCreate(&ctx->evb[i]) == hipSuccess;
  if (!ok) {
    izpi_gpu_close(ctx);
    return IZPI_ERR_HIP;
  }
  *out = ctx;
  return IZPI_OK;
}

int izpi_gpu_close(izpi_ctx* ctx) {
  if (!ctx) return IZPI_OK;
  (void)hipSetDevice(ctx->device);
  if (ctx->stream) (void)hipStreamSynchronize(ctx->stream);
  if (ctx->comm) (void)ncclCommDestroy(ctx->comm);
  free_scene(ctx);
  for (const CtxBuf& b : ctx_buffers(ctx)) if (*b.p) (void)hipFree(*b.p);
  void* fixed[] = {ctx->d_pool_ctr, ctx->d_misc, ctx->d_counters, ctx->d_status};
  for (void* p : fixed) if (p) (void)hipFree(p);
  if (ctx->h_count) (void)hipHostFree(ctx->h_count);
  if (ctx->stall_host) (void)hipHostFree(ctx->stall_host);
  for (int i = 0; i < 3 * IZPI_PASS_BATCH; i++) if (ctx->evb[i]) (void)hipEventDestroy(ctx->evb[i]);
  hipEvent_t evs[] = {ctx->ev0, ctx->ev1, ctx->ev2, ctx->ev3};
  for (hipEvent_t ev : evs) if (ev) (void)hipEventDestroy(ev);
  if (ctx->stream) (void)hipStreamDestroy(ctx->stream);
  delete ctx;
  return IZPI_OK;
}

const char* izpi_gpu_last_error(izpi_ctx* ctx) { return ctx ? ctx->err.c_str() : "null context"; }

int izpi_gpu_upload_scene(izpi_ctx* ctx, const izpi_scene_desc* d) {
  int rc = begin_upload(ctx, d);
  if (rc) return rc;
  PackedScene ps;
  rc = pack_scene(d, &ps, &ctx->err);
  return rc ? rc : upload_packed(ctx, d, ps);
}

uint64_t izpi_gpu_output_bytes(const izpi_render_req* req) {
  if (!req) return 0;
  if (req->out_layout == IZPI_OUT_PACKED && req->num_tiles) {
    uint64_t px = 0;
    for (uint32_t i = 0; i < req->num_tiles; i++) {
      const uint32_t* t = req->tiles + 4 * i;
      px += (uint64_t)(t[2] - t[0] + 1) * (t[3] - t[1] + 1);
    }
    return px * 4 * sizeof(double);
  }
  return (uint64_t)req->width * req->height * 4 * sizeof(double);
}

int izpi_gpu_render_device(izpi_ctx* ctx, const izpi_render_req* req, double* out_dev, izpi_render_stats* stats) {
  if (!ctx) return IZPI_ERR_INVALID;
  if (!out_dev) { ctx->err = "null output"; return IZPI_ERR_INVALID; }
  HIP_TRY(hipSetDevice(ctx->device));
  int rc = render_impl(ctx, req, one_shot(req), out_dev);
  if (stats) *stats = ctx->last;
  return rc;
}

int izpi_gpu_render(izpi_ctx* ctx, const izpi_render_req* req, double* out_host, izpi_render_stats* stats) {
  if (!ctx) return IZPI_ERR_INVALID;
  if (!out_host || !req) { ctx->err = "null argument"; return IZPI_ERR_INVALID; }
  if (session_open(ctx)) return IZPI_ERR_INVALID;
  HIP_TRY(hipSetDevice(ctx->device));
  const size_t bytes = izpi_gpu_output_bytes(req);
  int rc = grow(ctx, (void**)&ctx->d_out, &ctx->out_cap, bytes);
  if (rc) return rc;
  HIP_TRY(hipMemcpyAsync(ctx->d_out, out_host, bytes, hipMemcpyHostToDevice, ctx->stream));
  rc = render_impl(ctx, req, one_shot(req), ctx->d_out);
  if (stats) *stats = ctx->last;
  if (rc) return rc;
  HIP_TRY(hipMemcpyAsync(out_host, ctx->d_out, bytes, hipMemcpyDeviceToHost, ctx->stream));
  HIP_TRY(hipStreamSynchronize(ctx->stream));
  return IZPI_OK;
}

int izpi_gpu_prepare(izpi_ctx* ctx, const izpi_render_req* req) {
  if (!ctx) return IZPI_ERR_INVALID;
  if (!req) { ctx->err = "null argument"; return IZPI_ERR_INVALID; }
  if (session_open(ctx)) return IZPI_ERR_INVALID;
  HIP_TRY(hipSetDevice(ctx->device));
  if (ctx->comm && ctx->comm_size > 1) {
    Shares sh;
    int rc = make_shares(ctx, req, ctx->comm_size, sh);
    if (!rc) rc = share_buffers(ctx, sh, ctx->comm_rank == 0);
    return rc ? rc : render_share(ctx, req, sh, ctx->comm_rank, true);
  }
  return render_impl(ctx, req, one_shot(req, true), nullptr);
}

int izpi_gpu_progressive_begin_ex(izpi_ctx* ctx, const izpi_render_req* req, uint32_t step_spp, uint32_t flags) {
  if (!ctx) return IZPI_ERR_INVALID;
  HIP_TRY(hipSetDevice(ctx->device));
  return session_begin(ctx, req, step_spp, flags);
}

int izpi_gpu_progressive_begin(izpi_ctx* ctx, const izpi_render_req* req, uint32_t step_spp) {
  return izpi_gpu_progressive_begin_ex(ctx, req, step_spp, 0);
}

int izpi_gpu_progressive_noise(izpi_ctx* ctx, const izpi_noise_params* p, izpi_noise_stats* out) {
  if (!ctx) return IZPI_ERR_INVALID;
  HIP_TRY(hipSetDevice(ctx->device));
// ... 707 lines not shown
```

izpi_amd/csrc/izpi_kern.h:

```cpp
#pragma once
#include <hip/hip_runtime.h>
#include <stdio.h>
#include <stdlib.h>
#include <string.h>
#include <algorithm>
#include <cmath>
#include <string>
#include <vector>

#include <rccl/rccl.h>

#include <atomic>
#include <chrono>
#include <thread>

#include "../../include/izpi_host.h"
#include "../../include/izpi_gpu_debug.h"
#include "izpi_dev.h"
#include "izpi_req.h"
#include "render_plan.h"
#include "cie_tables.h"

using namespace izd;

#define HIP_TRY(expr)                                                                  \
  do {                                                                                 \
    hipError_t e_ = (expr);                                                            \
    if (e_ != hipSuccess) {                                                            \
      ctx->err = std::string(#expr) + ": " + hipGetErrorString(e_);                    \
      return IZPI_ERR_HIP;                                                             \
    }                                                                                  \
  } while (0)

static __constant__ double c_cie_wl[IZPI_CIE_N] = IZPI_CIE_WAVELENGTHS_INIT;
static __constant__ double c_cie_x[IZPI_CIE_N] = IZPI_CIE_X_INIT;
static __constant__ double c_cie_y[IZPI_CIE_N] = IZPI_CIE_Y_INIT;
static __constant__ double c_cie_z[IZPI_CIE_N] = IZPI_CIE_Z_INIT;
struct CieCum { double v[IZPI_CIE_N]; };
constexpr CieCum cie_y_running_sums() {
  CieCum c{};
  constexpr double y[IZPI_CIE_N] = IZPI_CIE_Y_INIT;
  double cur = 0.0;
  for (int i = 0; i < IZPI_CIE_N; i++) { c.v[i] = cur + y[i]; cur += y[i]; }
  return c;
}
static __constant__ CieCum c_cie_ycum = cie_y_running_sums();

namespace izpi_bvh {
int build(hipStream_t st, const double* h_boxes, uint32_t n, uint32_t leaf_max, uint32_t method,
          std::vector<izpi_bvh4_node>& nodes, std::vector<uint32_t>& order, float* ms, std::string& err);
}

#define IZPI_PASS_BATCH 8
constexpr uint32_t SHADE_THREADS = 256, SHADE_WAVES = SHADE_THREADS / 64;
constexpr uint32_t FINQ_WORDS = 5, FINQ_FLUSH = 1024, FINQ_CAP = FINQ_FLUSH + SHADE_THREADS;
constexpr int MISC_STRIDE = 64;

enum { CNT_RAYS = 0, CNT_NODES, CNT_TRI, CNT_SPH, CNT_LTRI, CNT_LSPH, CNT_NSTEP, CNT_PSTEP, CNT_SHORT,
       CNT_CLK_REFILL, CNT_CLK_NODE, CNT_CLK_PRIM, CNT_CLK_ADV, CNT_TAIL_NODES, CNT_TAIL_TRI, CNT_TAIL_SPH,
       CNT_SCLK_ITEM, CNT_SCLK_REFILL, CNT_SCLK_PUSH, CNT_PARK, CNT_SCLK_MAT, CNT_SCLK_FIN, CNT_SCLK_MIX, CNT_SCLK_LPDF,
       CNT_SCLK_ENTRY, CNT_SCLK_TEX, CNT_SCLK_RB1, CNT_SCLK_RATOM, CNT_SCLK_RB2,
       CNT_N };

IZPI_DEV void count_add(unsigned long long* cpart, unsigned long long* counters, int k, unsigned long long v) {
  if (v == 0) return;
  if (cpart) cpart[(size_t)__builtin_amdgcn_readfirstlane(blockIdx.x * (blockDim.x >> 6) + (threadIdx.x >> 6)) * CNT_N + k] += v;
  else atomicAdd(counters + k, v);
}

template <class T>
IZPI_DEV T sld(const T* p) { return *p; }
template <class T>
IZPI_DEV void sst(T* p, const T& v) { *p = v; }

template <class T>
IZPI_DEV T lds_ld(const T* p) {
  if constexpr (sizeof(T) % 8 == 0 && alignof(T) >= 8) {
    T r;
    uint64_t* d = reinterpret_cast<uint64_t*>(&r);
    const __attribute__((address_space(3))) uint64_t* q = (const __attribute__((address_space(3))) uint64_t*)p;
#pragma unroll
    for (uint32_t i = 0; i < sizeof(T) / 8; i++) d[i] = q[i];
    return r;
  } else {
    return *(const __attribute__((address_space(3))) T*)p;
  }
}

template <bool L, class T>
IZPI_DEV T tld(const T* p) {
  if constexpr (L) return lds_ld(p);
  else return *p;
}
constexpr uint32_t MAT_LDS = 64, TEX_LDS = 64, SPD_LDS = 384, BG_LDS = 128, MT_LDS = 64, LT_LDS = 64, PR_LDS = 64;
namespace lds_off {
constexpr uint32_t al(uint64_t b) { return (uint32_t)((b + 31) & ~31ull); }
constexpr uint32_t MC = 0;
constexpr uint32_t MT = MC + al(MT_LDS * sizeof(double4));
constexpr uint32_t LT = MT + al(MT_LDS * sizeof(MatTex));
constexpr uint32_t LT2 = LT + al(LT_LDS * 16 * sizeof(double));
constexpr uint32_t MAT = LT2 + al(LT_LDS * 6 * sizeof(double));
constexpr uint32_t TEX = MAT + al(MAT_LDS * sizeof(izpi_material));
constexpr uint32_t COLOUR_END = TEX + al(TEX_LDS * sizeof(izpi_texture));
constexpr uint32_t SPD = COLOUR_END;
constexpr uint32_t SPDV = SPD + al(SPD_LDS * sizeof(double));
constexpr uint32_t CIE = SPDV + al(SPD_LDS * sizeof(double));
constexpr uint32_t BG = CIE + al(5 * IZPI_CIE_N * sizeof(double));
constexpr uint32_t BGV = BG + al(BG_LDS * sizeof(double));
constexpr uint32_t SPECTRAL_END = BGV + al(BG_LDS * sizeof(double));
constexpr uint32_t GS = SPECTRAL_END;
constexpr uint32_t TT = GS + al(PR_LDS * sizeof(GShade));
constexpr uint32_t GP = TT + al(PR_LDS * sizeof(GTriTex));
constexpr uint32_t END = GP + al(PR_LDS * sizeof(GPrim));
constexpr uint32_t STG_RAY = COLOUR_END;
constexpr uint32_t STG_THR = STG_RAY + 3 * SHADE_THREADS * 16;
constexpr uint32_t STG_PATH = STG_THR + 3 * SHADE_THREADS * 8;
constexpr uint32_t STG_KIND = STG_PATH + SHADE_THREADS * 16;
constexpr uint32_t STG_END = STG_KIND + SHADE_THREADS * 4;
constexpr uint32_t STG_BYTES = STG_END - COLOUR_END;
}
IZPI_DEV char* lds_arena() {
  extern __shared__ __attribute__((aligned(16))) char izpi_lds_arena[];
  return izpi_lds_arena;
}
IZPI_DEV izpi_material* mat_lds() { return (izpi_material*)(lds_arena() + lds_off::MAT); }
IZPI_DEV izpi_texture* tex_lds() { return (izpi_texture*)(lds_arena() + lds_off::TEX); }
IZPI_DEV double* spd_lds() { return (double*)(lds_arena() + lds_off::SPD); }
IZPI_DEV double* spdv_lds() { return (double*)(lds_arena() + lds_off::SPDV); }
IZPI_DEV double* cie_lds() { return (double*)(lds_arena() + lds_off::CIE); }
IZPI_DEV double* bg_lds() { return (double*)(lds_arena() + lds_off::BG); }
IZPI_DEV double* bgv_lds() { return (double*)(lds_arena() + lds_off::BGV); }
IZPI_DEV izpi_material mat_rec(const DevScene& sc, bool st, uint32_t m) {
  if (st) return lds_ld(mat_lds() + m);
  return sc.materials[m];
}
IZPI_DEV izpi_texture tex_rec(const DevScene& sc, bool st, int32_t id) {
  if (st) return lds_ld(tex_lds() + id);
  return sc.textures[id];
}

IZPI_DEV V3 image_rgb(const double* texels, uint64_t off, uint32_t w, uint32_t h, uint32_t fmt, double u, double v) {
  int64_t i = go_int(u * (double)w);
  int64_t j = go_int((1 - v) * ((double)h - 0.001));
  if (i < 0) i = 0;
  if (j < 0) j = 0;
  if (i > (int64_t)w - 1) i = (int64_t)w - 1;
  if (j > (int64_t)h - 1) j = (int64_t)h - 1;
  uint64_t k = (uint64_t)j * w + (uint64_t)i;
  if (fmt == TEXF_GRAY) {
    const double g = texels[off + k];
    return mk(g, g, g);
  }
  const double* px = texels + off + k * 4;
  const double2 rg = *reinterpret_cast<const double2*>(px);
  return mk(rg.x, rg.y, px[2]);
}
IZPI_DEV uint64_t image_index(uint32_t w, uint32_t h, double u, double v) {
  int64_t i = go_int(u * (double)w);
  int64_t j = go_int((1 - v) * ((double)h - 0.001));
  if (i < 0) i = 0;
  if (j < 0) j = 0;
  if (i > (int64_t)w - 1) i = (int64_t)w - 1;
  if (j > (int64_t)h - 1) j = (int64_t)h - 1;
  return (uint64_t)j * w + (uint64_t)i;
}
IZPI_DEV V3 image_at(const double* texels, uint64_t off, uint32_t fmt, uint64_t k) {
  if (fmt == TEXF_GRAY) {
    const double g = texels[off + k];
    return mk(g, g, g);
  }
  const double* px = texels + off + k * 4;
  const double2 rg = *reinterpret_cast<const double2*>(px);
  return mk(rg.x, rg.y, px[2]);
}
IZPI_DEV V3 tex_rgb(const DevScene& sc, int32_t id, double u, double v, bool st = false) {
  const izpi_texture t = tex_rec(sc, st, id);
  if (t.kind == IZPI_TEX_IMAGE) return image_rgb(sc.texels, t.texel_offset, t.width, t.height, t.pad0, u, v);
  return mk(t.value[0], t.value[1], t.value[2]);
}
IZPI_DEV V3 slot_rgb(const DevScene& sc, const TexSlot& s, double u, double v, bool st = false) {
  const uint32_t fmt = s.hf >> 30;
  if (fmt <= TEXF_GRAY) return image_rgb(sc.texels, s.off, s.w, s.hf & 0x3FFFFFFFu, fmt, u, v);
  return tex_rgb(sc, (int32_t)s.off, u, v, st);
}
IZPI_DEV bool slot_set(const TexSlot& s) { return (s.hf >> 30) != TEXF_NONE; }
IZPI_DEV V3 slot_rgb_k(const DevScene& sc, const TexSlot& s, double u, double v, bool st, uint32_t w0, uint32_t h0, uint64_t k0) {
  const uint32_t fmt = s.hf >> 30, h = s.hf & 0x3FFFFFFFu;
  if (fmt <= TEXF_GRAY) {
    uint64_t k = k0;
    if (s.w != w0 || h != h0) k = image_index(s.w, h, u, v);
    return image_at(sc.texels, s.off, fmt, k);
  }
  return slot_rgb(sc, s, u, v, st);
}
IZPI_DEV MatTex* mt_lds() { return (MatTex*)(lds_arena() + lds_off::MT); }
IZPI_DEV TexSlot mat_slot(const DevScene& sc, bool staged, uint32_t m, int k) {
  if (staged) return lds_ld(&mt_lds()[m].s[k]);
  return sc.mat_tex[m].s[k];
}
template <bool L = false>
IZPI_DEV uint32_t sorted_interval(const double* wl, uint32_t n, double w) {
  uint32_t lo = 1, hi = n - 1;
  while (lo < hi) {
    const uint32_t mid = (lo + hi) >> 1;
    if (tld<L>(wl + mid) >= w) hi = mid; else lo = mid + 1;
  }
  return lo - 1;
}

IZPI_DEV double spectral_image_value(double r, double g, double b, double wl) {
  double sv = 0;
  if (wl >= 580.0 && wl <= 750.0) {
    const double dist = gm::abs(wl - 650.0);
    sv += r * gm::exp(-(dist * dist) / (2.0 * 60.0 * 60.0));
  }
// ... 959 lines not shown
  using Tail = void (*)(DevScene, ShadeParams, WaveParams, int32_t*);
  Shade shade, shade_staged;
  Tail tail32, tail64;
  Shade start;
  void (*refill)(DevScene, ShadeParams, WaveParams, const uint32_t*);
  uint32_t sampler, rec_doubles;
  int matset;
  bool fwd;
  char name[24];
};
template <int SAMPLER, bool FWD>
const ShadeKernels* shade_kernels(int matset);

struct SampleRange {
  uint32_t begin, end;
  bool keep;
};
struct ResolveParams {
  uint32_t num_pixels, done, width, height, tile_w, tile_h, sampler, out_layout;
  uint32_t form;
  double exposure;
  const uint32_t* tiles;
  const double* running;
  double* out;
};
void launch_resolve(hipStream_t st, const ResolveParams& rp);
struct NoiseParams {
  uint32_t num_pixels, done, width, height, tile_w, tile_h, sampler, out_layout;
  double threshold, floor;
  const uint32_t* tiles;
  const double* running;
  const double* moments;
  double* out;
  double* block_sums;
  unsigned long long* block_counts;
};
void launch_noise_resolve(hipStream_t st, const NoiseParams& np);
void launch_noise_stats(hipStream_t st, const NoiseParams& np);
static_assert(sizeof(RayOD) == izpi_internal::plan_size::RAY && sizeof(PathHot) == izpi_internal::plan_size::PATH_HOT &&
                  sizeof(PathCold) == izpi_internal::plan_size::PATH_COLD && sizeof(double2) == izpi_internal::plan_size::HIT,
              "render_plan.h: entry records");
static_assert(SMP_D == izpi_internal::plan_size::SMP_D && POOL_SHARDS == izpi_internal::plan_size::POOL_SHARDS,
              "render_plan.h: per-sample results, pool rings");
static_assert(RecLayout<IZPI_SAMPLER_COLOUR, MATSET_FULL>::D == izpi_internal::plan_size::REC_COLOUR &&
                  RecLayout<IZPI_SAMPLER_COLOUR, MATSET_CONST>::D == izpi_internal::plan_size::REC_COMPACT &&
                  RecLayout<IZPI_SAMPLER_SPECTRAL, MATSET_FULL>::D == izpi_internal::plan_size::REC_SPECTRAL,
              "render_plan.h: record strides");
struct DevBufs {
  std::vector<void*> p;
  template <typename T>
  hipError_t alloc(T** out, size_t count) {
    *out = nullptr;
    const hipError_t e = hipMalloc((void**)out, count * sizeof(T));
    if (e == hipSuccess) p.push_back(*out);
    return e;
  }
  ~DevBufs() {
    for (void* q : p) (void)hipFree(q);
  }
};

struct izpi_ctx {
  int device = 0;
  std::string err;
  hipStream_t stream = nullptr;
  hipEvent_t ev0 = nullptr, ev1 = nullptr, ev2 = nullptr;
  int num_cus = 0;
  bool have_scene = false;
  uint32_t num_textures = 0;
  uint32_t num_materials = 0;
  uint32_t num_spd = 0;
  izpi_internal::PlanCache plans[2];
  const GTriVerts* d_triverts = nullptr;
  DevScene sc{};
  uint32_t stack_needed = 0;
  uint32_t num_prims = 0;
  std::vector<void*> scene_allocs;
  size_t scene_bytes = 0;
  double* d_samples = nullptr; size_t samples_cap = 0;
  double* d_recs = nullptr; size_t recs_cap = 0;
  double* d_pool = nullptr; size_t pool_cap = 0;
  uint32_t* d_ring = nullptr; size_t ring_cap = 0;
  unsigned long long* d_pool_ctr = nullptr;
  double* d_running = nullptr; size_t running_cap = 0;
  double* d_out = nullptr; size_t out_cap = 0;
  uint32_t* d_tiles = nullptr; size_t tiles_cap = 0;
  uint32_t* d_utiles = nullptr; size_t utiles_cap = 0;
  double* d_bg = nullptr; size_t bg_cap = 0;
  uint32_t* d_misc = nullptr;
  unsigned long long* d_counters = nullptr;
  unsigned long long* d_cpart = nullptr; size_t cpart_cap = 0;
  unsigned long long* d_finq = nullptr; size_t finq_cap = 0;
  char* d_state = nullptr; size_t state_cap = 0;
  int32_t* d_spill = nullptr; size_t spill_cap = 0;
  double* d_post = nullptr; size_t post_cap = 0;
  double* d_share = nullptr; size_t share_cap = 0;
  double* d_gather = nullptr; size_t gather_cap = 0;
  double* d_denoise = nullptr; size_t denoise_cap = 0;
  double* d_moments = nullptr; size_t moments_cap = 0;
  double* d_noisepart = nullptr; size_t noisepart_cap = 0;
  uint32_t* h_count = nullptr;
  hipEvent_t ev3 = nullptr;
  hipEvent_t evb[3 * IZPI_PASS_BATCH] = {};
  ncclComm_t comm = nullptr;
  volatile uint32_t* stall_word = nullptr;
  uint32_t* stall_host = nullptr;
  uint32_t comm_rank = 0, comm_size = 1;
  int32_t* d_status = nullptr;
  int fault_inject = 0;
  izpi_render_stats last{};
  bool mat_ok_rgb = false, mat_ok_spectral = false;
  bool basic_materials = false;
  uint32_t matset = 0;
  bool const_albedo = false;
  bool any_uv = false;
  const ShadeKernels* kernels[2][2] = {};
  uint32_t pool_grow = 0;
  uint32_t dev_share = 1;
  std::atomic<uint64_t> prog_done{0}, prog_total{0};
  struct Session {
    bool open = false;
    bool broken = false;
    izpi_render_req req{};
    izpi_render_tuning tuning{};
    std::vector<uint32_t> tiles;
    std::vector<double> bg_wl, bg_val;
    uint32_t step_spp = 0, done = 0;
    bool noise = false;
    std::vector<uint32_t> run_tiles;
    uint32_t tile_w = 0, tile_h = 0, num_pixels = 0;
    izpi_render_stats cum{};
  } session;
};

inline uint32_t* misc(izpi_ctx* ctx, int k) { return ctx->d_misc + (size_t)k * MISC_STRIDE; }

template <typename K>
inline int resident_blocks(izpi_ctx* ctx, K kernel, int* blocks, int threads = 256, size_t dyn_lds = 0) {
  int per_cu = 0;
  if (dyn_lds) HIP_TRY(hipFuncSetAttribute((const void*)kernel, hipFuncAttributeMaxDynamicSharedMemorySize, (int)dyn_lds));
  HIP_TRY(hipOccupancyMaxActiveBlocksPerMultiprocessor(&per_cu, kernel, threads, dyn_lds));
  if (per_cu < 1) per_cu = 1;
  *blocks = per_cu * ctx->num_cus;
  return IZPI_OK;
}

constexpr int TRACE_RING = 16, TRACE_WPE = 5;
struct Tracer {
  bool p2 = true;
  bool tri = false;
  bool lds_bvh = false;
  bool ray_lds = false;
  bool qnodes = false;
  uint32_t prim_w = 32, tchunk = 512, refill_min = 24;
  int blocks = 0;
  size_t spill_bytes = 0;
};

const izpi_render_tuning kDefaultTuning{};

int make_tracer(izpi_ctx* ctx, const izpi_render_tuning& tu, bool need_uv, Tracer* t);
void launch_trace(izpi_ctx* ctx, const DevScene& sc, const Tracer& t, const WaveParams& wp, hipStream_t st, int32_t* spill);
struct RunInput { uint32_t num_pixels, chunk, pool_blocks; SampleRange range; };
struct RunTimes { float trace_ms = 0, shade_ms = 0, tail_ms = 0; uint32_t launches = 0; };
const ShadeKernels* shade_instance(uint32_t matset, bool const_basic, uint32_t sampler, bool fwd);
int run_wavefront(izpi_ctx* ctx, const izpi_render_req* req, const DevScene& sc, const Tracer& tr, const ShadeKernels& k,
                  ShadeParams& sp, WaveParams& wp, AccumParams& ap, const RunInput& in, RunTimes* out);
int prepare_wavefront(izpi_ctx* ctx, const ShadeKernels& k);
int prepare_accumulate(izpi_ctx* ctx);
void launch_accumulate(hipStream_t st, const AccumParams& ap, double* moments = nullptr);
inline double* session_moments(const izpi_ctx* ctx, const SampleRange& r) {
  return r.keep && ctx->session.noise ? ctx->d_moments : nullptr;
}
struct PreviewParams {
  WaveBuf buf;
  double2* tminmax;
  const GTriVerts* verts;
  double ink[3];
  uint32_t slots;
};
int run_preview(izpi_ctx* ctx, const izpi_render_req* req, const DevScene& sc, const Tracer& tr, ShadeParams& sp,
                const PreviewParams& pp, AccumParams& ap, const RunInput& in, RunTimes* out);
int prepare_preview(izpi_ctx* ctx);
inline bool preview_sampler(uint32_t s) {
  return s == IZPI_SAMPLER_NORMAL || s == IZPI_SAMPLER_ALBEDO || s == IZPI_SAMPLER_WIREFRAME;
}
inline double diag_clock_ms() {
  return std::chrono::duration<double, std::milli>(std::chrono::steady_clock::now().time_since_epoch()).count();
}
```

izpi_amd/csrc/scene_pack.h:

```cpp
#pragma once
#include <stddef.h>
#include <stdint.h>
#include <string>
#include <vector>

#include "scene_records.h"

namespace izpi_internal {

struct Double4 { double x, y, z, w; };

struct PackedScene {
  std::vector<izd::GInner> inner;
  std::vector<izd::GInnerQ> innerq;
  std::vector<izd::GLeaf> leaves;
  std::vector<izd::GPrim> prims;
  std::vector<izd::GShade> shade;
  std::vector<izd::GTriVerts> triverts;
  std::vector<izd::GTriTex> tritex;
  std::vector<izd::GLight> lights;
  std::vector<Double4> mat_const;
  std::vector<izd::MatTex> mat_tex;
  std::vector<izpi_texture> textures;
  std::vector<double> texels;
  int32_t root = -1;
  uint32_t num_inner = 0, leaf_shortcut = 1, quantized = 0, nan_free_bounds = 1, time_free = 1, no_pathlen = 1, tri_only = 1;
  uint32_t stack_needed = 0;
  bool mat_ok_rgb = true, mat_ok_spectral = true;
  bool basic_materials = true;
  uint32_t matset = 0;
  bool const_albedo = true;
  bool any_uv = false;
};

int pack_scene(const izpi_scene_desc* d, PackedScene* out, std::string* err);

bool stack_bound(const izpi_bvh4_node* nodes, size_t n, uint32_t* bound);

}
```

izpi_amd/csrc/trace.hip:

```cpp
#include "izpi_kern.h"

constexpr uint32_t BVH_LDS_BYTES = 4096;
__device__ __forceinline__ bool lane_of(uint64_t mask) { return __builtin_amdgcn_inverse_ballot_w64(mask); }
__device__ __forceinline__ uint32_t lanes_below(uint64_t mask) {
  return __builtin_amdgcn_mbcnt_hi((uint32_t)(mask >> 32), __builtin_amdgcn_mbcnt_lo((uint32_t)mask, 0u));
}
template <int S, int WPE, bool DIST, bool TRI, bool LB, bool RL, bool Q>
__global__ void __launch_bounds__(256) __attribute__((amdgpu_waves_per_eu(WPE))) k_trace2(const DevScene sc, const WaveParams wp, unsigned long long* counters,
                                                uint32_t* err, int32_t* spill, uint32_t spill_stride, uint32_t prim_w,
                                                uint32_t tchunk, uint32_t refill_min) {
  static_assert((S & (S - 1)) == 0, "ring size must be a power of two");
  static_assert(!LB || DIST, "the LDS-resident BVH instance runs the distributed leaf tests");
  static_assert(!RL || (DIST && (TRI || LB)), "the LDS-resident ray instances: triangle-only global BVH, or the BVH in LDS");
  static_assert(!Q || !LB, "the quantised nodes are read from global memory");
  constexpr bool UVL = !RL, UVS = RL && LB, DUV = !RL || LB;
  typedef float v4f __attribute__((ext_vector_type(4)));
  typedef double v2d __attribute__((ext_vector_type(2)));
  typedef const __attribute__((address_space(3))) v4f LF4;
  typedef const __attribute__((address_space(3))) v2d LD2;
  __shared__ float4 bvh_lds[LB ? BVH_LDS_BYTES / 16 : 1];
  LF4* const l_inner = (LF4*)bvh_lds;
  LF4* const l_leaves = l_inner + (size_t)8 * (LB ? sc.num_inner : 0);
  LD2* const l_prims = (LD2*)(l_leaves + (size_t)2 * (LB ? sc.num_prims : 0));
  if constexpr (LB) {
    const uint32_t ni = 8 * sc.num_inner, nl = 2 * sc.num_prims, np5 = 5 * sc.num_prims;
    for (uint32_t t = threadIdx.x; t < ni + nl + np5; t += 256)
      bvh_lds[t] = t < ni ? reinterpret_cast<const float4*>(sc.inner)[t]
                          : (t < ni + nl ? reinterpret_cast<const float4*>(sc.leaves)[t - ni]
                                         : reinterpret_cast<const float4*>(sc.prims)[t - ni - nl]);
    __syncthreads();
  }
  __shared__ int32_t lds_stack[S * 256];
  __shared__ uint32_t dist_owner[DIST ? 260 : 1];
  __shared__ double dist_t[DIST ? 260 : 1], dist_u[DIST && DUV ? 260 : 1], dist_v[DIST && DUV ? 260 : 1];
  __shared__ double2 lds_uv[UVL ? 256 : 1];
  __shared__ double2 ray_lds[RL ? 3 * 256 : 1];
  const uint32_t wbase = threadIdx.x & ~63u;
  int32_t* stk = lds_stack + threadIdx.x;
  int32_t* gsp = spill + blockIdx.x * 256 + threadIdx.x;
  const uint32_t lane = threadIdx.x & 63;
  const uint32_t n = *wp.in_count;
  if (wp.pool_ctr && blockIdx.x == 0) pool_publish(wp.pool_ctr);
  if (wp.out_count && blockIdx.x == 0 && threadIdx.x == 0) *wp.out_count = 0;
  if (wp.out_park && blockIdx.x == 0 && threadIdx.x == 0) *wp.out_park = 0;
  const bool read_kind = wp.read_kind != 0 || (wp.in_park && *wp.in_park != 0);
  const uint32_t nwaves = gridDim.x * 4u;
  const uint32_t chunk = min(tchunk, max(16u, (n + nwaves - 1u) / nwaves));
  const uint32_t first = chunk;
  if ((uint64_t)(blockIdx.x * 4u + (threadIdx.x >> 6)) * first >= n) return;
  uint64_t c_rays = 0, c_nodes = 0, c_tri = 0, c_sph = 0;
  uint64_t c_nstep = 0, c_pstep = 0, c_short = 0;
  bool busy = false, in_prim = false;
  bool exhausted = false;
  uint32_t qi = 0;
  uint32_t lkind = RAY_MAIN;
  double tmax = 0;
  float ix = 0, iy = 0, iz = 0, ox = 0, oy = 0, oz = 0;
  int32_t cur = -1, pk = 0, pend = 0;
  int sp = -1, low = 0;
  int clean_from = 0;
  int32_t bprim = -1;
  bool fast = false;
  uint64_t m_slow = ~0ull;
  bool any_spill = false;
#ifdef IZPI_SHADOW
  uint64_t c_spill_st = 0, c_spill_ld = 0;
  uint32_t sh_acc = 0;
#endif
  uint32_t c_pos = __builtin_amdgcn_readfirstlane((blockIdx.x * 4u + (threadIdx.x >> 6)) * first);
  uint32_t c_end = c_pos + first < n ? c_pos + first : n;
#ifdef IZPI_TRACE_CLOCKS
  uint64_t k_refill = 0, k_node = 0, k_prim = 0, k_adv = 0, k0 = 0, k1 = 0;
#define IZPI_CLK(v) (v) = __builtin_readcyclecounter()
#else
#define IZPI_CLK(v) (void)0
#endif
#ifdef IZPI_STEP_MARKS
#define IZPI_MARK(name) asm volatile("; IZPI_MARK " name)
#else
#define IZPI_MARK(name) (void)0
#endif
  for (;;) {
    IZPI_CLK(k0);
    IZPI_MARK("head");
    const uint64_t idle = __builtin_amdgcn_ballot_w64(sp < 0);
    uint64_t idle_now = idle;
    if (idle != 0) {
      const uint32_t nidle = (uint32_t)__popcll(idle);
      if (!exhausted && (nidle >= refill_min || idle == ~0ull) && c_pos >= c_end) {
        IZPI_MARK("dequeue");
        uint32_t b = 0;
        if (lane == 0) b = atomicAdd(wp.trace_next, chunk);
        b = __builtin_amdgcn_readfirstlane(b) + nwaves * first;
        if (b >= n) exhausted = true;
        c_pos = b;
        c_end = b + chunk < n ? b + chunk : n;
      }
      if (!exhausted && (nidle >= refill_min || idle == ~0ull) && c_pos < c_end) {
        IZPI_MARK("refill");
        const uint32_t take = nidle < c_end - c_pos ? nidle : c_end - c_pos;
        const uint32_t base = c_pos;
        c_pos += take;
        bool main_ray = false;
        const uint32_t rank = lanes_below(idle);
        const uint32_t my = base + rank;
        if (!busy && rank < take) {
          const uint32_t k = read_kind ? sld(wp.in.kind + my) : (uint32_t)RAY_MAIN;
          RayOD r;
          if constexpr (RL) {
            r = sld(wp.in.ray + my);
            const double2* rp = reinterpret_cast<const double2*>(&r);
            const double2 r0 = rp[0], r1 = rp[1], r2 = rp[2];
            ray_lds[3 * threadIdx.x] = r0; ray_lds[3 * threadIdx.x + 1] = r1; ray_lds[3 * threadIdx.x + 2] = r2;
          } else {
            r = wp.in.ray[my];
          }
          if (!(k & (RAY_PARKED | RAY_DEAD)) && (uint64_t)__double_as_longlong(r.o[0]) != DEAD_BITS) {
            qi = my;
            lkind = k;
            tmax = ray_tmax(wp.in, my, k);
            main_ray = kind_of(k) == RAY_MAIN;
            ix = (float)(1.0 / r.d[0]); iy = (float)(1.0 / r.d[1]); iz = (float)(1.0 / r.d[2]);
            ox = (float)r.o[0]; oy = (float)r.o[1]; oz = (float)r.o[2];
            fast = sc.nan_free_bounds && ray_fast_ok(ox, oy, oz, ix, iy, iz);
            cur = sc.root;
            busy = cur != -1;
            sp = busy ? 0 : -1; low = 0; clean_from = 0;
            in_prim = false;
            bprim = -1;
            if (!busy) {
              if ((UVL || UVS) && wp.hit_uv) {
                double2* rec = wp.in.hit + ((size_t)my << 1);
                sst(rec, hit_pack(0.0, -1)); sst(rec + 1, make_double2(0.0, 0.0));
              } else {
                sst(wp.in.hit + my, hit_pack(0.0, -1));
              }
            }
          }
        }
        c_rays += (uint64_t)__popcll(__ballot(main_ray));
        m_slow = __ballot(!fast);
        idle_now = __builtin_amdgcn_ballot_w64(sp < 0);
        __builtin_amdgcn_s_waitcnt(0x0F70);
      } else if (exhausted && idle == ~0ull) {
        break;
      }
    }
    IZPI_MARK("pick");
    const uint64_t m_prim = __builtin_amdgcn_ballot_w64(pk < pend);
    const uint64_t m_node = ~(m_prim | idle_now);
    if ((m_prim | m_node) == 0) continue;
    const uint32_t n_prim = (uint32_t)__popcll(m_prim), n_node = (uint32_t)__popcll(m_node);
    bool advance = false;
    bool leaf_next = false;
    int32_t next = -1;
#ifdef IZPI_TRACE_CLOCKS
    IZPI_CLK(k1); k_refill += k1 - k0; k0 = k1;
    const bool clk_prim = n_prim * prim_w >= n_node * 16u;
#endif
    if (n_prim * prim_w >= n_node * 16u) {
      if constexpr (DIST) {
        IZPI_MARK("prim");
        const uint32_t cnt = (uint32_t)(pend - pk);
        const uint32_t base = lanes_below(__ballot(cnt & 1u)) + 2u * lanes_below(__ballot(cnt & 2u)) +
                              4u * lanes_below(__ballot(cnt & 4u));
        const uint64_t ms = m_prim & __builtin_amdgcn_ballot_w64(base + cnt <= 64);
        const bool served = lane_of(ms);
        const int last = 63 - __clzll((long long)ms);
        const uint32_t total = (uint32_t)__builtin_amdgcn_readlane((int)(base + cnt), last);
        {
          const uint32_t e = ((uint32_t)pk << 6) | lane;
          uint32_t* dq = dist_owner + wbase + base;
          if (served) dq[0] = e;
          if (served && cnt > 1) dq[1] = e + 64u;
          if (served && cnt > 2) dq[2] = e + 128u;
          if (served && cnt > 3) dq[3] = e + 192u;
        }
        __builtin_amdgcn_wave_barrier();
        const uint32_t ent = lane < total ? dist_owner[wbase + lane] : lane;
        const uint32_t ow = ent & 63u;
        const uint32_t oqi = (uint32_t)__shfl((int)qi, (int)ow);
        const uint32_t okind = (uint32_t)__shfl((int)lkind, (int)ow);
        if (lane < total) {
          const int32_t pi = (int32_t)(ent >> 6);
          double2 r0, r1, r2;
          if constexpr (RL) {
            const uint32_t ro = 3 * (wbase + ow);
            r0 = ray_lds[ro]; r1 = ray_lds[ro + 1]; r2 = ray_lds[ro + 2];
          } else {
            const double2* rp = reinterpret_cast<const double2*>(wp.in.ray + oqi);
            r0 = rp[0]; r1 = rp[1]; r2 = rp[2];
          }
          const double otmin = ray_tmin(wp.in, oqi, okind);
          double2 p0, p1, p2, p3, p4;
          if constexpr (LB) {
            LD2* pp = l_prims + (size_t)5 * pi;
            const v2d a0 = pp[0], a1 = pp[1], a2 = pp[2], a3 = pp[3], a4 = pp[4];
            p0 = make_double2(a0.x, a0.y); p1 = make_double2(a1.x, a1.y); p2 = make_double2(a2.x, a2.y);
            p3 = make_double2(a3.x, a3.y); p4 = make_double2(a4.x, a4.y);
          } else {
            const double2* pp = reinterpret_cast<const double2*>(sc.prims + pi);
            p0 = pp[0]; p1 = pp[1]; p2 = pp[2]; p3 = pp[3]; p4 = pp[4];
#ifdef IZPI_SHADOW
            if (IZPI_SHADOW & 4) {
              const uint4* sq = reinterpret_cast<const uint4*>(sc.sh_prims + pi);
              const uint4 s0 = sq[0], s1 = sq[1], s2 = sq[2], s3 = sq[3], s4 = sq[4];
              sh_acc ^= s0.x ^ s1.y ^ s2.z ^ s3.w ^ s4.x;
            }
#endif
          }
          const double pa[9] = {p0.x, p0.y, p1.x, p1.y, p2.x, p2.y, p3.x, p3.y, p4.x};
          double t = 0, u = 0, v = 0;
          const V3 o = mk(r0.x, r0.y, r1.x), d = mk(r1.y, r2.x, r2.y);
          uint32_t flags;
          if (TRI || (uint32_t)__double2loint(p4.y) == IZPI_PRIM_TRIANGLE) {
            flags = tri_intersect_no_tmax(pa, o, d, otmin, t, u, v) ? 1u : 0u;
          } else {
            const double time = (RL && LB) || sc.time_free ? pa[7] : (wp.in.time ? wp.in.time[oqi] : 0.0);
            flags = 2u;
            if (sph_roots(sph_center(pa, time), pa[6], o, d, t, u))
              flags |= 1u | (t > otmin ? 4u : 0u) | (u > otmin ? 8u : 0u);
          }
          dist_t[wbase + lane] = t;
          if constexpr (DUV) { dist_u[wbase + lane] = u; dist_v[wbase + lane] = v; }
          dist_owner[wbase + lane] = flags;
        }
        const uint32_t n_sph_tests = TRI ? 0u : (uint32_t)__popcll(__ballot(lane < total && (dist_owner[wbase + lane] & 2u)));
        __builtin_amdgcn_wave_barrier();
        if (served && (TRI || n_sph_tests == 0)) {
          const uint32_t j0 = wbase + base;
          uint32_t f[4];
          double tt[4];
#pragma unroll
          for (uint32_t i = 0; i < 4; i++) { f[i] = dist_owner[j0 + i]; tt[i] = dist_t[j0 + i]; }
          int32_t acc = -1;
#pragma unroll
          for (uint32_t i = 0; i < 4; i++)
            if (i < cnt && (f[i] & 1u) && !(tt[i] > tmax)) { tmax = tt[i]; acc = (int32_t)i; }
          if (acc >= 0) {
            if constexpr (UVL) lds_uv[threadIdx.x] = make_double2(dist_u[j0 + acc], dist_v[j0 + acc]);
            if constexpr (UVS)
              if (wp.hit_uv) sst(wp.in.hit + ((size_t)qi << 1) + 1, make_double2(dist_u[j0 + acc], dist_v[j0 + acc]));
            bprim = pk + acc;
            clean_from = sp;
          }
          pk = pend;
          in_prim = false;
          advance = true;
        } else if (!TRI && served) {
          int32_t acc = -1;
          double acc_u = 0, acc_v = 0;
          for (uint32_t i = 0; i < cnt; i++) {
            const uint32_t j = wbase + base + i;
            const uint32_t f = dist_owner[j];
            if (!(f & 1u)) continue;
            if (!(f & 2u)) {
              const double t = dist_t[j];
              if (!(t > tmax)) { tmax = t; acc = (int32_t)j; acc_u = dist_u[j]; acc_v = dist_v[j]; bprim = pk + (int32_t)i; }
            } else {
              const double ta = dist_t[j], tb = dist_u[j];
              if (ta < tmax && (f & 4u)) { tmax = ta; acc = (int32_t)j; acc_u = 0.0; acc_v = 0.0; bprim = pk + (int32_t)i; }
              else if (tb < tmax && (f & 8u)) { tmax = tb; acc = (int32_t)j; acc_u = 1.0; acc_v = 0.0; bprim = pk + (int32_t)i; }
            }
          }
          if (acc >= 0) {
            if constexpr (UVS) {
              if (wp.hit_uv) sst(wp.in.hit + ((size_t)qi << 1) + 1, make_double2(acc_u, acc_v));
            } else {
              lds_uv[threadIdx.x] = make_double2(acc_u, acc_v);
            }
            clean_from = sp;
          }
          pk = pend;
          in_prim = false;
          advance = true;
        }
        __builtin_amdgcn_wave_barrier();
        c_tri += total - n_sph_tests;
        c_sph += n_sph_tests;
        c_pstep++;
      } else {
      bool is_tri = false;
      if (busy && in_prim) {
        const double2* rp = reinterpret_cast<const double2*>(wp.in.ray + qi);
        const double2 r0 = rp[0], r1 = rp[1], r2 = rp[2];
        const V3 o = mk(r0.x, r0.y, r1.x), d = mk(r1.y, r2.x, r2.y);
        const double tmin = ray_tmin(wp.in, qi, lkind);
        const double2* pp = reinterpret_cast<const double2*>(sc.prims + pk);
        const double2 p0 = pp[0], p1 = pp[1], p2 = pp[2], p3 = pp[3], p4 = pp[4];
        const double pa[9] = {p0.x, p0.y, p1.x, p1.y, p2.x, p2.y, p3.x, p3.y, p4.x};
        is_tri = TRI || (uint32_t)__double2loint(p4.y) == IZPI_PRIM_TRIANGLE;
        if (is_tri) {
          double t, u, v;
          if (tri_intersect(pa, o, d, tmin, tmax, t, u, v)) {
            tmax = t; bprim = pk; lds_uv[threadIdx.x] = make_double2(u, v); clean_from = sp;
          }
        } else if (!TRI) {
          const double time = wp.in.time ? wp.in.time[qi] : 0.0;
          double t; int root;
          if (sph_intersect(pa, o, d, time, tmin, tmax, t, root)) {
            tmax = t; bprim = pk; lds_uv[threadIdx.x] = make_double2((double)root, 0.0); clean_from = sp;
          }
        }
        pk++;
        if (pk == pend) { in_prim = false; advance = true; }
      }
      const uint32_t n_tri = (uint32_t)__popcll(__ballot(is_tri));
      c_tri += n_tri;
      c_sph += n_prim - n_tri;
      c_pstep++;
      }
    } else {
      IZPI_MARK("node");
      c_nodes += n_node;
      c_nstep++;
      const bool wave_fast = (m_node & m_slow) == 0;
      if ((m_node & __builtin_amdgcn_ballot_w64(sp + 3 - low > S)) != 0) {
        any_spill = true;
        if (busy && !in_prim) {
          while (sp + 3 - low > S) {
            gsp[(size_t)low * spill_stride] = stk[(low & (S - 1)) * 256];
            low++;
#ifdef IZPI_SHADOW
            c_spill_st++;
#endif
          }
        }
      }
      if (busy && !in_prim) {
        const float tm = (float)tmax;
        const bool is_leaf = ref_is_leaf(cur);
        float4 q0, q1, mnz_, mxx_, mxy_, mxz_;
        int4 ch_;
        if constexpr (LB) {
          LF4* lp = is_leaf ? l_leaves + (size_t)2 * leaf_start(cur) : l_inner + (size_t)8 * cur;
          LF4* np = is_leaf ? l_inner : lp;
          const v4f a0 = lp[0], a1 = lp[1], a2 = np[2], a3 = np[3], a4 = np[4], a5 = np[5], c = np[6];
          q0 = make_float4(a0.x, a0.y, a0.z, a0.w); q1 = make_float4(a1.x, a1.y, a1.z, a1.w);
          mnz_ = make_float4(a2.x, a2.y, a2.z, a2.w); mxx_ = make_float4(a3.x, a3.y, a3.z, a3.w);
          mxy_ = make_float4(a4.x, a4.y, a4.z, a4.w); mxz_ = make_float4(a5.x, a5.y, a5.z, a5.w);
          ch_ = make_int4(__float_as_int(c.x), __float_as_int(c.y), __float_as_int(c.z), __float_as_int(c.w));
        } else if constexpr (Q) {
          const float4* lp = reinterpret_cast<const float4*>(is_leaf ? (const void*)(sc.leaves + leaf_start(cur))
                                                                     : (const void*)(sc.innerq + cur));
          const float4* np = is_leaf ? reinterpret_cast<const float4*>(sc.innerq) : lp;
          q0 = lp[0]; q1 = lp[1];
          const float4 c2 = np[2], c3 = np[3];
          const uint32_t ex = __float_as_uint(q0.w);
          const float sx = __uint_as_float((ex & 0xFFu) << 23), sy = __uint_as_float(((ex >> 8) & 0xFFu) << 23),
                      sz = __uint_as_float(((ex >> 16) & 0xFFu) << 23);
          auto dec4 = [](float w, float o, float sc_) {
            const uint32_t b = __float_as_uint(w);
            return make_float4(__builtin_fmaf((float)(b & 0xFFu), sc_, o), __builtin_fmaf((float)((b >> 8) & 0xFFu), sc_, o),
                               __builtin_fmaf((float)((b >> 16) & 0xFFu), sc_, o), __builtin_fmaf((float)(b >> 24), sc_, o));
          };
          const float4 dmnx = dec4(q1.x, q0.x, sx), dmny = dec4(q1.y, q0.y, sy), dmnz = dec4(q1.z, q0.z, sz);
          const float4 dmxx = dec4(q1.w, q0.x, sx), dmxy = dec4(c2.x, q0.y, sy), dmxz = dec4(c2.y, q0.z, sz);
          const float4 l0 = q0, l1 = q1;
          q0 = is_leaf ? l0 : dmnx;
          q1 = is_leaf ? l1 : make_float4(dmny.x, dmny.y, dmny.z, dmny.w);
          mnz_ = dmnz; mxx_ = dmxx; mxy_ = dmxy; mxz_ = dmxz;
          ch_ = make_int4(__float_as_int(c2.z), __float_as_int(c2.w), __float_as_int(c3.x), __float_as_int(c3.y));
        } else {
          const float4* lp = reinterpret_cast<const float4*>(is_leaf ? (const void*)(sc.leaves + leaf_start(cur))
                                                                     : (const void*)(sc.inner + cur));
          const float4* np = is_leaf ? reinterpret_cast<const float4*>(sc.inner) : lp;
          q0 = lp[0]; q1 = lp[1];
          mnz_ = np[2]; mxx_ = np[3]; mxy_ = np[4]; mxz_ = np[5];
          ch_ = *reinterpret_cast<const int4*>(np + 6);
#ifdef IZPI_SHADOW
          if ((IZPI_SHADOW & 1) && !is_leaf) {
            const uint4* sq = reinterpret_cast<const uint4*>(sc.sh_inner + cur);
            const uint4 s0 = sq[0], s1 = sq[1], s2 = sq[2], s3 = sq[3], s4 = sq[4], s5 = sq[5], s6 = sq[6];
            sh_acc ^= s0.x ^ s1.y ^ s2.z ^ s3.w ^ s4.x ^ s5.y ^ s6.z;
          }
          if ((IZPI_SHADOW & 2) && is_leaf) {
            const uint4* sq = reinterpret_cast<const uint4*>(sc.sh_leaves + leaf_start(cur));
            const uint4 s0 = sq[0], s1 = sq[1];
            sh_acc ^= s0.x ^ s1.y;
          }
#endif
        }
        const float4 mnx = q0;
        const float4 mny = make_float4(is_leaf ? q0.y : q1.x, q1.y, q1.z, q1.w);
        const float4 mnz = make_float4(is_leaf ? q0.z : mnz_.x, mnz_.y, mnz_.z, mnz_.w);
        const float4 mxx = make_float4(is_leaf ? q0.w : mxx_.x, mxx_.y, mxx_.z, mxx_.w);
        const float4 mxy = make_float4(is_leaf ? q1.x : mxy_.x, mxy_.y, mxy_.z, mxy_.w);
        const float4 mxz = make_float4(is_leaf ? q1.y : mxz_.x, mxz_.y, mxz_.z, mxz_.w);
        const int4 ch = make_int4(is_leaf ? cur : ch_.x, ch_.y, ch_.z, ch_.w);
        uint64_t hit[4];
        if (wave_fast) {
          slab4_fast(mnx, mny, mnz, mxx, mxy, mxz, ox, oy, oz, ix, iy, iz, tm, hit);
        } else {
          const float amnx[4] = {mnx.x, mnx.y, mnx.z, mnx.w}, amny[4] = {mny.x, mny.y, mny.z, mny.w},
                      amnz[4] = {mnz.x, mnz.y, mnz.z, mnz.w}, amxx[4] = {mxx.x, mxx.y, mxx.z, mxx.w},
                      amxy[4] = {mxy.x, mxy.y, mxy.z, mxy.w}, amxz[4] = {mxz.x, mxz.y, mxz.z, mxz.w};
#pragma unroll
          for (int i = 0; i < 4; i++)
            hit[i] = __builtin_amdgcn_ballot_w64(slab(amnx[i], amny[i], amnz[i], amxx[i], amxy[i], amxz[i], ox, oy, oz, ix, iy, iz, tm));
        }
        const uint64_t m_inner = __builtin_amdgcn_ballot_w64(cur >= -1);
        const uint64_t b0 = hit[0] & __builtin_amdgcn_ballot_w64(ch.x != -1),
                       b1 = hit[1] & m_inner & __builtin_amdgcn_ballot_w64(ch.y != -1),
                       b2 = hit[2] & m_inner & __builtin_amdgcn_ballot_w64(ch.z != -1),
                       b3 = hit[3] & m_inner & __builtin_amdgcn_ballot_w64(ch.w != -1);
        next = lane_of(b3) ? ch.w : -1;
        next = lane_of(b2) ? ch.z : next;
        next = lane_of(b1) ? ch.y : next;
        next = lane_of(b0) ? ch.x : next;
        const bool enter = ref_is_leaf(next) && (is_leaf || sc.leaf_shortcut);
        leaf_next = enter && !is_leaf;
        in_prim = enter;
        pk = enter ? leaf_start(next) : pk;
        pend = enter ? leaf_start(next) + leaf_count(next) : pend;
        next = enter ? -1 : next;
        const uint64_t r1 = b0 & b1, r2 = (b0 | b1) & b2, r3 = (b0 | b1 | b2) & b3;
        const int np_ = (int)lane_of(r1) + (int)lane_of(r2) + (int)lane_of(r3);
        const int32_t e0z = lane_of(r2) ? ch.z : ch.w;
        const int32_t e0 = lane_of(r1) ? ch.y : e0z;
        const int32_t e1 = lane_of(r1 & r2) ? ch.z : ch.w;
        stk[(sp & (S - 1)) * 256] = e0;
        stk[((sp + 1) & (S - 1)) * 256] = e1;
        stk[((sp + 2) & (S - 1)) * 256] = ch.w;
        if (sp + np_ > 64) atomicOr(err, 1u);
        sp += np_;
        advance = !enter;
      }
    }
#ifdef IZPI_TRACE_CLOCKS
    IZPI_CLK(k1); if (clk_prim) k_prim += k1 - k0; else k_node += k1 - k0; k0 = k1;
#endif
    {
      IZPI_MARK("advance");
      const bool do_pop = advance && next == -1 && sp > 0;
      const bool do_fin = advance && next == -1 && sp == 0;
      const int spn = sp - 1;
      int32_t top = *(volatile __attribute__((address_space(3))) int32_t*)&lds_stack[threadIdx.x + (spn & (S - 1)) * 256];
      if (any_spill && __ballot(do_pop && spn < low) != 0) {
        if (do_pop && spn < low) {
          top = gsp[(size_t)spn * spill_stride];
          low = spn;
#ifdef IZPI_SHADOW
          c_spill_ld++;
#endif
        }
        __builtin_amdgcn_s_waitcnt(0x0F70);
      }
      cur = (advance && next != -1) ? next : (do_pop ? top : cur);
      sp = (advance && next == -1) ? spn : sp;
      const bool lf = do_pop && ref_is_leaf(top) && spn >= clean_from && sc.leaf_shortcut;
      in_prim = in_prim || lf;
      leaf_next = leaf_next || lf;
      pk = lf ? leaf_start(top) : pk;
      pend = lf ? leaf_start(top) + leaf_count(top) : pend;
      clean_from = (do_pop && spn < clean_from) ? spn : clean_from;
      if (do_fin) {
        const double2 uv = (UVL && bprim >= 0) ? lds_uv[threadIdx.x] : make_double2(0.0, 0.0);
        if ((UVL || UVS) && wp.hit_uv) {
          double2* rec = wp.in.hit + ((size_t)qi << 1);
          sst(rec, hit_pack(bprim >= 0 ? tmax : 0.0, bprim));
          if (!UVS || bprim < 0) sst(rec + 1, uv);
        } else {
          sst(wp.in.hit + qi, hit_pack(bprim >= 0 ? tmax : 0.0, bprim));
        }
        busy = false;
      }
    }
    const uint64_t n_short = (uint64_t)__popcll(__ballot(leaf_next));
    c_nodes += n_short;
    c_short += n_short;
#ifdef IZPI_TRACE_CLOCKS
    IZPI_CLK(k1); k_adv += k1 - k0;
#endif
  }
#ifdef IZPI_TRACE_CLOCKS
  if (lane == 0) {
    atomicAdd(counters + CNT_CLK_REFILL, (unsigned long long)k_refill);
    atomicAdd(counters + CNT_CLK_NODE, (unsigned long long)k_node);
    atomicAdd(counters + CNT_CLK_PRIM, (unsigned long long)k_prim);
    atomicAdd(counters + CNT_CLK_ADV, (unsigned long long)k_adv);
  }
#endif
#ifdef IZPI_SHADOW
  {
    if (c_spill_st) atomicAdd(counters + CNT_CLK_REFILL, (unsigned long long)c_spill_st);
    if (c_spill_ld) atomicAdd(counters + CNT_CLK_NODE, (unsigned long long)c_spill_ld);
    if (sh_acc == 0x9E3779B9u) atomicOr(err, 0u);
  }
#endif
  if (lane == 0) {
    count_add(wp.cpart, counters, CNT_RAYS, c_rays);
    count_add(wp.cpart, counters, CNT_NODES, c_nodes);
    count_add(wp.cpart, counters, CNT_TRI, c_tri);
    count_add(wp.cpart, counters, CNT_SPH, c_sph);
    count_add(wp.cpart, counters, CNT_NSTEP, c_nstep);
    count_add(wp.cpart, counters, CNT_PSTEP, c_pstep);
    count_add(wp.cpart, counters, CNT_SHORT, c_short);
  }
}


#define IZPI_T2_LIST(X)                                                                                           \
  X(true, false, false, false, false) X(true, true, false, false, false) X(false, false, false, false, false)        \
  X(false, true, false, false, false) X(true, false, true, false, false) X(true, true, true, false, false)           \
  X(true, true, false, true, false) X(true, false, true, true, false) X(true, true, true, true, false)               \
  X(true, false, false, false, true) X(true, true, false, false, true) X(true, true, false, true, true)
constexpr int ring_of(bool lb, bool rl) { return lb && rl ? 8 : TRACE_RING; }

int make_tracer(izpi_ctx* ctx, const izpi_render_tuning& tu, bool need_uv, Tracer* t) {
  *t = Tracer();
  if (tu.flags & IZPI_TUNE_NO_DIST) t->p2 = false;
  if (ctx->num_prims >= (1u << 26)) t->p2 = false;
  t->tri = ctx->sc.tri_only != 0 && !(tu.flags & IZPI_TUNE_GENERAL_TRACE);
  t->lds_bvh = t->p2 && !(tu.flags & IZPI_TUNE_NO_LDS_BVH) &&
               (uint64_t)ctx->sc.num_inner * sizeof(GInner) + (uint64_t)ctx->sc.num_prims * (sizeof(GLeaf) + sizeof(GPrim)) <= BVH_LDS_BYTES;
  if (t->lds_bvh) {
    t->refill_min = 40;
    t->prim_w = 24;
  }
  t->ray_lds = t->p2 && ((t->tri && !t->lds_bvh && !need_uv) || (t->lds_bvh && (t->tri || ctx->sc.time_free))) &&
               !(tu.flags & IZPI_TUNE_NO_RAY_LDS);
  t->qnodes = ctx->sc.quantized && t->p2 && !t->lds_bvh && !(tu.flags & IZPI_TUNE_NO_QNODES);
  if (tu.prim_weight) t->prim_w = tu.prim_weight;
  if (tu.trace_chunk) t->tchunk = tu.trace_chunk;
  if (tu.refill_min) t->refill_min = std::min<uint32_t>(64, tu.refill_min);
  int rc = IZPI_ERR_INVALID;
  ctx->err = "no k_trace2 instance for this scene and tuning";
#define IZPI_T2_OCC(P, T, L, R, Q)                                                               \
  if (t->p2 == P && t->tri == T && t->lds_bvh == L && t->ray_lds == R && t->qnodes == Q) \
    rc = resident_blocks(ctx, k_trace2<ring_of(L, R), TRACE_WPE, P, T, L, R, Q>, &t->blocks);
  IZPI_T2_LIST(IZPI_T2_OCC)
#undef IZPI_T2_OCC
  if (rc) return rc;
  t->spill_bytes = (size_t)t->blocks * 256 * 64 * sizeof(int32_t);
  return IZPI_OK;
}

void launch_trace(izpi_ctx* ctx, const DevScene& sc, const Tracer& t, const WaveParams& wp, hipStream_t st, int32_t* spill) {
  const dim3 g(t.blocks), b(256);
  const uint32_t stride = (uint32_t)t.blocks * 256;
#define IZPI_T2_LAUNCH(P, T, L, R, Q)                                                                          \
  if (t.p2 == P && t.tri == T && t.lds_bvh == L && t.ray_lds == R && t.qnodes == Q) {                          \
    hipLaunchKernelGGL((k_trace2<ring_of(L, R), TRACE_WPE, P, T, L, R, Q>), g, b, 0, st, sc, wp, ctx->d_counters, \
                       misc(ctx, 1), spill, stride, t.prim_w, t.tchunk, t.refill_min);                        \
    return;                                                                                                    \
  }
  IZPI_T2_LIST(IZPI_T2_LAUNCH)
#undef IZPI_T2_LAUNCH
}
```

Baseline: 2593.

## Address BVH nodes, leaves and prims with 32-bit offsets from one base

Places inner nodes, quantised nodes and leaves in one contiguous device allocation and adds a kernel template flag that addresses them, and the primitive records, through 32-bit byte offsets from a shared base pointer instead of 64-bit pointer arithmetic. The distributed traversal also keeps a single packed leaf reference per lane in place of separate start and end indices. Both changes aim to cut VGPR use and 64-bit address instructions in the traversal loop, at the cost of twice as many kernel instantiations. Optional instruction-count instrumentation and extra marker points are added for profiling.

```diff
diff --git a/include/izpi_gpu.h b/include/izpi_gpu.h
--- a/include/izpi_gpu.h
+++ b/include/izpi_gpu.h
@@ -86,7 +86,8 @@
   IZPI_TUNE_NO_PRIM_LDS = 256,
   IZPI_TUNE_NO_PLACE_PICK = 512,
   IZPI_TUNE_NO_QNODES = 1024,
-  IZPI_TUNE_NO_SHADE_STAGE = 2048
+  IZPI_TUNE_NO_SHADE_STAGE = 2048,
+  IZPI_TUNE_WIDE_ADDR = 4096
 };
 
 typedef struct izpi_render_req {
diff --git a/izpi_amd/_native.py b/izpi_amd/_native.py
--- a/izpi_amd/_native.py
+++ b/izpi_amd/_native.py
@@ -96,6 +96,7 @@
 TUNE_NO_PRIM_LDS = 256
 TUNE_NO_QNODES = 1024
 TUNE_NO_SHADE_STAGE = 2048
+TUNE_WIDE_ADDR = 4096
 
 
 def tuning(**kw):
diff --git a/izpi_amd/csrc/izpi_dev.h b/izpi_amd/csrc/izpi_dev.h
--- a/izpi_amd/csrc/izpi_dev.h
+++ b/izpi_amd/csrc/izpi_dev.h
@@ -36,6 +36,7 @@
   uint32_t lds_bytes;
   uint32_t time_free;
   uint32_t quantized;
+  uint32_t addr32;
 #ifdef IZPI_SHADOW
   const GInner* sh_inner;
   const GLeaf* sh_leaves;
diff --git a/izpi_amd/csrc/izpi_gpu.hip b/izpi_amd/csrc/izpi_gpu.hip
--- a/izpi_amd/csrc/izpi_gpu.hip
+++ b/izpi_amd/csrc/izpi_gpu.hip
@@ -7,6 +7,9 @@
 using izpi_internal::Double4;
 using izpi_internal::pack_scene;
 using izpi_internal::PackedScene;
+using izpi_internal::trace_addr32;
+using izpi_internal::trace_layout;
+using izpi_internal::TraceLayout;
 using izpi_internal::PlanCache;
 using izpi_internal::PlanInput;
 using izpi_internal::SideLayout;
@@ -591,8 +594,8 @@
   const double t_tiles = host_ms();
   if ((rc = make_tracer(ctx, tu, !ctx->sc.tri_only || ctx->any_uv, &tr))) return rc;
   if (pass_log)
-    fprintf(stderr, "IZPI_TRACE_INSTANCE dist=%d tri=%d lds_bvh=%d ray_lds=%d q=%d\n", (int)tr.p2, (int)tr.tri, (int)tr.lds_bvh,
-            (int)tr.ray_lds, (int)tr.qnodes);
+    fprintf(stderr, "IZPI_TRACE_INSTANCE dist=%d tri=%d lds_bvh=%d ray_lds=%d q=%d\nIZPI_TRACE_ADDR a32=%d ring=%d\n", (int)tr.p2, (int)tr.tri,
+            (int)tr.lds_bvh, (int)tr.ray_lds, (int)tr.qnodes, (int)(tr.a32 && !tr.lds_bvh), trace_ring(tr));
   const double t_tracer = host_ms();
   PlanCache& cache = ctx->plans[rs.preview];
   PlanInput in = plan_input(ctx, req, rs, tu, call.size_spp);
@@ -680,6 +683,12 @@
 #ifdef IZPI_SHADOW
   fprintf(stderr, "IZPI_SHADOW spill_stores %llu spill_loads %llu (entries)\n", cnt[CNT_CLK_REFILL], cnt[CNT_CLK_NODE]);
 #endif
+#ifdef IZPI_TRACE_ICOUNT
+  fprintf(stderr, "IZPI_TRACE_ICOUNT {\"iterations\": %llu, \"idle\": %llu, \"dequeue\": %llu, \"refill\": %llu, \"prim\": %llu, \"node_fast\": %llu, "
+          "\"node_twin\": %llu, \"spill\": %llu, \"readback\": %llu, \"pop\": %llu, \"finish\": %llu, \"waves\": %llu}\n",
+          cnt[CNT_IC_ITER], cnt[CNT_IC_IDLE], cnt[CNT_IC_DEQUEUE], cnt[CNT_IC_REFILL], cnt[CNT_PSTEP], cnt[CNT_NSTEP] - cnt[CNT_IC_TWIN], cnt[CNT_IC_TWIN],
+          cnt[CNT_IC_SPILL], cnt[CNT_IC_READBACK], cnt[CNT_IC_POP], cnt[CNT_IC_FINISH], cnt[CNT_IC_WAVES]);
+#endif
 #ifdef IZPI_TRACE_CLOCKS
   fprintf(stderr, "IZPI_TRACE_CLOCKS refill %llu node %llu prim %llu advance %llu (wave cycles)\n", cnt[CNT_CLK_REFILL],
           cnt[CNT_CLK_NODE], cnt[CNT_CLK_PRIM], cnt[CNT_CLK_ADV]);
@@ -1034,9 +1043,17 @@
   GInner* di; GInnerQ* dq; GLeaf* dl; GPrim* dp; GShade* dsh; GTriVerts* dtv; GTriTex* dtt; GLight* dlt;
   izpi_material* dm; Double4* dmc; MatTex* dmt; izpi_texture* dtx;
   double *dtex, *dswl, *dsv;
-  UP(ps.inner.data(), ps.inner.size(), &di);
-  UP(ps.innerq.data(), ps.innerq.size(), &dq);
-  UP(ps.leaves.data(), ps.leaves.size(), &dl);
+  {
+    const TraceLayout tl = trace_layout(ps.inner.size(), ps.innerq.size(), ps.leaves.size());
+    char* nb;
+    UP((const char*)nullptr, tl.bytes, &nb);
+    di = reinterpret_cast<GInner*>(nb);
+    dq = ps.innerq.empty() ? nullptr : reinterpret_cast<GInnerQ*>(nb + tl.innerq_at);
+    dl = reinterpret_cast<GLeaf*>(nb + tl.leaves_at);
+    HIP_TRY(hipMemcpy(di, ps.inner.data(), ps.inner.size() * sizeof(GInner), hipMemcpyHostToDevice));
+    if (dq) HIP_TRY(hipMemcpy(dq, ps.innerq.data(), ps.innerq.size() * sizeof(GInnerQ), hipMemcpyHostToDevice));
+    HIP_TRY(hipMemcpy(dl, ps.leaves.data(), ps.leaves.size() * sizeof(GLeaf), hipMemcpyHostToDevice));
+  }
   UP(ps.prims.data(), ps.prims.size(), &dp);
   UP(ps.shade.data(), ps.shade.size(), &dsh);
   UP(ps.triverts.data(), ps.triverts.size(), &dtv);
@@ -1064,6 +1081,7 @@
   sc.root = ps.root; sc.num_inner = ps.num_inner; sc.num_prims = d->num_prims; sc.num_lights = d->num_lights;
   sc.quantized = ps.quantized; sc.leaf_shortcut = ps.leaf_shortcut; sc.nan_free_bounds = ps.nan_free_bounds;
   sc.tri_only = ps.tri_only; sc.time_free = ps.time_free; sc.no_pathlen = ps.no_pathlen;
+  sc.addr32 = trace_addr32(ps.inner.size(), ps.innerq.size(), ps.leaves.size(), ps.prims.size());
   sc.cam = d->camera;
   ctx->d_triverts = dtv;
   ctx->mat_ok_rgb = ps.mat_ok_rgb; ctx->mat_ok_spectral = ps.mat_ok_spectral;
diff --git a/izpi_amd/csrc/izpi_kern.h b/izpi_amd/csrc/izpi_kern.h
--- a/izpi_amd/csrc/izpi_kern.h
+++ b/izpi_amd/csrc/izpi_kern.h
@@ -61,6 +61,14 @@
        CNT_SCLK_ITEM, CNT_SCLK_REFILL, CNT_SCLK_PUSH, CNT_PARK, CNT_SCLK_MAT, CNT_SCLK_FIN, CNT_SCLK_MIX, CNT_SCLK_LPDF,
        CNT_SCLK_ENTRY, CNT_SCLK_TEX, CNT_SCLK_RB1, CNT_SCLK_RATOM, CNT_SCLK_RB2,
        CNT_N };
+#ifdef IZPI_TRACE_ICOUNT
+enum { CNT_IC_ITER = CNT_CLK_REFILL, CNT_IC_DEQUEUE = CNT_CLK_NODE, CNT_IC_REFILL = CNT_CLK_PRIM, CNT_IC_TWIN = CNT_CLK_ADV,
+       CNT_IC_SPILL = CNT_SCLK_ITEM, CNT_IC_READBACK = CNT_SCLK_REFILL, CNT_IC_POP = CNT_SCLK_PUSH, CNT_IC_FINISH = CNT_SCLK_MAT,
+       CNT_IC_WAVES = CNT_SCLK_FIN, CNT_IC_IDLE = CNT_SCLK_MIX };
+#if defined(IZPI_TRACE_CLOCKS) || defined(IZPI_SHADE_CLOCKS) || defined(IZPI_SHADOW)
+#error "IZPI_TRACE_ICOUNT shares counter rows with the clock and shadow builds"
+#endif
+#endif
 
 IZPI_DEV void count_add(unsigned long long* cpart, unsigned long long* counters, int k, unsigned long long v) {
   if (v == 0) return;
@@ -1326,6 +1334,7 @@
   bool lds_bvh = false;
   bool ray_lds = false;
   bool qnodes = false;
+  bool a32 = false;
   uint32_t prim_w = 32, tchunk = 512, refill_min = 24;
   int blocks = 0;
   size_t spill_bytes = 0;
@@ -1335,6 +1344,7 @@
 
 int make_tracer(izpi_ctx* ctx, const izpi_render_tuning& tu, bool need_uv, Tracer* t);
 void launch_trace(izpi_ctx* ctx, const DevScene& sc, const Tracer& t, const WaveParams& wp, hipStream_t st, int32_t* spill);
+int trace_ring(const Tracer& t);
 struct RunInput { uint32_t num_pixels, chunk, pool_blocks; SampleRange range; };
 struct RunTimes { float trace_ms = 0, shade_ms = 0, tail_ms = 0; uint32_t launches = 0; };
 const ShadeKernels* shade_instance(uint32_t matset, bool const_basic, uint32_t sampler, bool fwd);
diff --git a/izpi_amd/csrc/scene_pack.h b/izpi_amd/csrc/scene_pack.h
--- a/izpi_amd/csrc/scene_pack.h
+++ b/izpi_amd/csrc/scene_pack.h
@@ -35,6 +35,19 @@
 
 int pack_scene(const izpi_scene_desc* d, PackedScene* out, std::string* err);
 
+struct TraceLayout { uint64_t innerq_at, leaves_at, bytes; };
+inline TraceLayout trace_layout(uint64_t n_inner, uint64_t n_innerq, uint64_t n_leaves) {
+  TraceLayout t;
+  t.innerq_at = n_inner * sizeof(izd::GInner);
+  t.leaves_at = t.innerq_at + n_innerq * sizeof(izd::GInnerQ);
+  t.bytes = t.leaves_at + n_leaves * sizeof(izd::GLeaf);
+  return t;
+}
+inline bool trace_addr32(uint64_t n_inner, uint64_t n_innerq, uint64_t n_leaves, uint64_t n_prims) {
+  const uint64_t lim = 1ull << 32;
+  return trace_layout(n_inner, n_innerq, n_leaves).bytes <= lim && n_prims * sizeof(izd::GPrim) <= lim;
+}
+
 bool stack_bound(const izpi_bvh4_node* nodes, size_t n, uint32_t* bound);
 
 }
diff --git a/izpi_amd/csrc/trace.hip b/izpi_amd/csrc/trace.hip
--- a/izpi_amd/csrc/trace.hip
+++ b/izpi_amd/csrc/trace.hip
@@ -5,7 +5,7 @@
 __device__ __forceinline__ uint32_t lanes_below(uint64_t mask) {
   return __builtin_amdgcn_mbcnt_hi((uint32_t)(mask >> 32), __builtin_amdgcn_mbcnt_lo((uint32_t)mask, 0u));
 }
-template <int S, int WPE, bool DIST, bool TRI, bool LB, bool RL, bool Q>
+template <int S, int WPE, bool DIST, bool TRI, bool LB, bool RL, bool Q, bool A32>
 __global__ void __launch_bounds__(256) __attribute__((amdgpu_waves_per_eu(WPE))) k_trace2(const DevScene sc, const WaveParams wp, unsigned long long* counters,
                                                 uint32_t* err, int32_t* spill, uint32_t spill_stride, uint32_t prim_w,
                                                 uint32_t tchunk, uint32_t refill_min) {
@@ -13,6 +13,7 @@
   static_assert(!LB || DIST, "the LDS-resident BVH instance runs the distributed leaf tests");
   static_assert(!RL || (DIST && (TRI || LB)), "the LDS-resident ray instances: triangle-only global BVH, or the BVH in LDS");
   static_assert(!Q || !LB, "the quantised nodes are read from global memory");
+  static_assert(!A32 || !LB, "the 32-bit offsets address records in global memory");
   constexpr bool UVL = !RL, UVS = RL && LB, DUV = !RL || LB;
   typedef float v4f __attribute__((ext_vector_type(4)));
   typedef double v2d __attribute__((ext_vector_type(2)));
@@ -36,6 +37,10 @@
   __shared__ double2 lds_uv[UVL ? 256 : 1];
   __shared__ double2 ray_lds[RL ? 3 * 256 : 1];
   const uint32_t wbase = threadIdx.x & ~63u;
+  constexpr uint32_t NODE_BYTES = Q ? sizeof(GInnerQ) : sizeof(GInner);
+  const char* const nbase = Q ? reinterpret_cast<const char*>(sc.innerq) : reinterpret_cast<const char*>(sc.inner);
+  const char* const pbase = reinterpret_cast<const char*>(sc.prims);
+  const uint32_t leaf_off0 = A32 ? (uint32_t)(reinterpret_cast<const char*>(sc.leaves) - nbase) : 0u;
   int32_t* stk = lds_stack + threadIdx.x;
   int32_t* gsp = spill + blockIdx.x * 256 + threadIdx.x;
   const uint32_t lane = threadIdx.x & 63;
@@ -57,6 +62,7 @@
   double tmax = 0;
   float ix = 0, iy = 0, iz = 0, ox = 0, oy = 0, oz = 0;
   int32_t cur = -1, pk = 0, pend = 0;
+  int32_t lref = 0;
   int sp = -1, low = 0;
   int clean_from = 0;
   int32_t bprim = -1;
@@ -80,15 +86,25 @@
 #else
 #define IZPI_MARK(name) (void)0
 #endif
+#ifdef IZPI_TRACE_ICOUNT
+  uint32_t ic_iter = 0, ic_idle = 0, ic_dequeue = 0, ic_refill = 0, ic_twin = 0, ic_spill = 0, ic_readback = 0, ic_pop = 0, ic_finish = 0;
+#define IZPI_IC(v) (v)++
+#else
+#define IZPI_IC(v) (void)0
+#endif
   for (;;) {
     IZPI_CLK(k0);
     IZPI_MARK("head");
+    IZPI_IC(ic_iter);
     const uint64_t idle = __builtin_amdgcn_ballot_w64(sp < 0);
     uint64_t idle_now = idle;
     if (idle != 0) {
+      IZPI_MARK("idle");
+      IZPI_IC(ic_idle);
       const uint32_t nidle = (uint32_t)__popcll(idle);
       if (!exhausted && (nidle >= refill_min || idle == ~0ull) && c_pos >= c_end) {
         IZPI_MARK("dequeue");
+        IZPI_IC(ic_dequeue);
         uint32_t b = 0;
         if (lane == 0) b = atomicAdd(wp.trace_next, chunk);
         b = __builtin_amdgcn_readfirstlane(b) + nwaves * first;
@@ -98,6 +114,7 @@
       }
       if (!exhausted && (nidle >= refill_min || idle == ~0ull) && c_pos < c_end) {
         IZPI_MARK("refill");
+        IZPI_IC(ic_refill);
         const uint32_t take = nidle < c_end - c_pos ? nidle : c_end - c_pos;
         const uint32_t base = c_pos;
         c_pos += take;
@@ -147,7 +164,7 @@
       }
     }
     IZPI_MARK("pick");
-    const uint64_t m_prim = __builtin_amdgcn_ballot_w64(pk < pend);
+    const uint64_t m_prim = DIST ? __builtin_amdgcn_ballot_w64(lref < 0) : __builtin_amdgcn_ballot_w64(pk < pend);
     const uint64_t m_node = ~(m_prim | idle_now);
     if ((m_prim | m_node) == 0) continue;
     const uint32_t n_prim = (uint32_t)__popcll(m_prim), n_node = (uint32_t)__popcll(m_node);
@@ -161,7 +178,8 @@
     if (n_prim * prim_w >= n_node * 16u) {
       if constexpr (DIST) {
         IZPI_MARK("prim");
-        const uint32_t cnt = (uint32_t)(pend - pk);
+        const uint32_t cnt = lref < 0 ? (uint32_t)leaf_count(lref) : 0u;
+        pk = leaf_start(lref);
         const uint32_t base = lanes_below(__ballot(cnt & 1u)) + 2u * lanes_below(__ballot(cnt & 2u)) +
                               4u * lanes_below(__ballot(cnt & 4u));
         const uint64_t ms = m_prim & __builtin_amdgcn_ballot_w64(base + cnt <= 64);
@@ -199,7 +217,8 @@
             p0 = make_double2(a0.x, a0.y); p1 = make_double2(a1.x, a1.y); p2 = make_double2(a2.x, a2.y);
             p3 = make_double2(a3.x, a3.y); p4 = make_double2(a4.x, a4.y);
           } else {
-            const double2* pp = reinterpret_cast<const double2*>(sc.prims + pi);
+            const double2* pp = A32 ? reinterpret_cast<const double2*>(pbase + (uint32_t)pi * (uint32_t)sizeof(GPrim))
+                                    : reinterpret_cast<const double2*>(sc.prims + pi);
             p0 = pp[0]; p1 = pp[1]; p2 = pp[2]; p3 = pp[3]; p4 = pp[4];
 #ifdef IZPI_SHADOW
             if (IZPI_SHADOW & 4) {
@@ -244,7 +263,7 @@
             bprim = pk + acc;
             clean_from = sp;
           }
-          pk = pend;
+          lref = 0;
           in_prim = false;
           advance = true;
         } else if (!TRI && served) {
@@ -271,7 +290,7 @@
             }
             clean_from = sp;
           }
-          pk = pend;
+          lref = 0;
           in_prim = false;
           advance = true;
         }
@@ -286,7 +305,8 @@
         const double2 r0 = rp[0], r1 = rp[1], r2 = rp[2];
         const V3 o = mk(r0.x, r0.y, r1.x), d = mk(r1.y, r2.x, r2.y);
         const double tmin = ray_tmin(wp.in, qi, lkind);
-        const double2* pp = reinterpret_cast<const double2*>(sc.prims + pk);
+        const double2* pp = A32 ? reinterpret_cast<const double2*>(pbase + (uint32_t)pk * (uint32_t)sizeof(GPrim))
+                                : reinterpret_cast<const double2*>(sc.prims + pk);
         const double2 p0 = pp[0], p1 = pp[1], p2 = pp[2], p3 = pp[3], p4 = pp[4];
         const double pa[9] = {p0.x, p0.y, p1.x, p1.y, p2.x, p2.y, p3.x, p3.y, p4.x};
         is_tri = TRI || (uint32_t)__double2loint(p4.y) == IZPI_PRIM_TRIANGLE;
@@ -315,8 +335,13 @@
       c_nodes += n_node;
       c_nstep++;
       const bool wave_fast = (m_node & m_slow) == 0;
+#ifdef IZPI_TRACE_ICOUNT
+      if (!wave_fast) ic_twin++;
+#endif
       if ((m_node & __builtin_amdgcn_ballot_w64(sp + 3 - low > S)) != 0) {
+        IZPI_MARK("spill");
         any_spill = true;
+        IZPI_IC(ic_spill);
         if (busy && !in_prim) {
           while (sp + 3 - low > S) {
             gsp[(size_t)low * spill_stride] = stk[(low & (S - 1)) * 256];
@@ -327,23 +352,32 @@
           }
         }
       }
+      IZPI_MARK("node_loads");
       if (busy && !in_prim) {
         const float tm = (float)tmax;
         const bool is_leaf = ref_is_leaf(cur);
         float4 q0, q1, mnz_, mxx_, mxy_, mxz_;
         int4 ch_;
+        const float4 *lp = nullptr, *np = nullptr;
+        if constexpr (!LB && A32) {
+          const uint32_t noff = is_leaf ? 0u : (uint32_t)cur * NODE_BYTES;
+          const uint32_t loff = is_leaf ? leaf_off0 + (uint32_t)leaf_start(cur) * (uint32_t)sizeof(GLeaf) : noff;
+          lp = reinterpret_cast<const float4*>(nbase + loff);
+          np = reinterpret_cast<const float4*>(nbase + noff);
+        } else if constexpr (!LB) {
+          lp = reinterpret_cast<const float4*>(is_leaf ? (const void*)(sc.leaves + leaf_start(cur))
+                                                       : Q ? (const void*)(sc.innerq + cur) : (const void*)(sc.inner + cur));
+          np = is_leaf ? reinterpret_cast<const float4*>(nbase) : lp;
+        }
         if constexpr (LB) {
-          LF4* lp = is_leaf ? l_leaves + (size_t)2 * leaf_start(cur) : l_inner + (size_t)8 * cur;
-          LF4* np = is_leaf ? l_inner : lp;
-          const v4f a0 = lp[0], a1 = lp[1], a2 = np[2], a3 = np[3], a4 = np[4], a5 = np[5], c = np[6];
+          LF4* llp = is_leaf ? l_leaves + (size_t)2 * leaf_start(cur) : l_inner + (size_t)8 * cur;
+          LF4* lnp = is_leaf ? l_inner : llp;
+          const v4f a0 = llp[0], a1 = llp[1], a2 = lnp[2], a3 = lnp[3], a4 = lnp[4], a5 = lnp[5], c = lnp[6];
           q0 = make_float4(a0.x, a0.y, a0.z, a0.w); q1 = make_float4(a1.x, a1.y, a1.z, a1.w);
           mnz_ = make_float4(a2.x, a2.y, a2.z, a2.w); mxx_ = make_float4(a3.x, a3.y, a3.z, a3.w);
           mxy_ = make_float4(a4.x, a4.y, a4.z, a4.w); mxz_ = make_float4(a5.x, a5.y, a5.z, a5.w);
           ch_ = make_int4(__float_as_int(c.x), __float_as_int(c.y), __float_as_int(c.z), __float_as_int(c.w));
         } else if constexpr (Q) {
-          const float4* lp = reinterpret_cast<const float4*>(is_leaf ? (const void*)(sc.leaves + leaf_start(cur))
-                                                                     : (const void*)(sc.innerq + cur));
-          const float4* np = is_leaf ? reinterpret_cast<const float4*>(sc.innerq) : lp;
           q0 = lp[0]; q1 = lp[1];
           const float4 c2 = np[2], c3 = np[3];
           const uint32_t ex = __float_as_uint(q0.w);
@@ -362,9 +396,6 @@
           mnz_ = dmnz; mxx_ = dmxx; mxy_ = dmxy; mxz_ = dmxz;
           ch_ = make_int4(__float_as_int(c2.z), __float_as_int(c2.w), __float_as_int(c3.x), __float_as_int(c3.y));
         } else {
-          const float4* lp = reinterpret_cast<const float4*>(is_leaf ? (const void*)(sc.leaves + leaf_start(cur))
-                                                                     : (const void*)(sc.inner + cur));
-          const float4* np = is_leaf ? reinterpret_cast<const float4*>(sc.inner) : lp;
           q0 = lp[0]; q1 = lp[1];
           mnz_ = np[2]; mxx_ = np[3]; mxy_ = np[4]; mxz_ = np[5];
           ch_ = *reinterpret_cast<const int4*>(np + 6);
@@ -390,8 +421,10 @@
         const int4 ch = make_int4(is_leaf ? cur : ch_.x, ch_.y, ch_.z, ch_.w);
         uint64_t hit[4];
         if (wave_fast) {
+          IZPI_MARK("slab_fast");
           slab4_fast(mnx, mny, mnz, mxx, mxy, mxz, ox, oy, oz, ix, iy, iz, tm, hit);
         } else {
+          IZPI_MARK("slab_twin");
           const float amnx[4] = {mnx.x, mnx.y, mnx.z, mnx.w}, amny[4] = {mny.x, mny.y, mny.z, mny.w},
                       amnz[4] = {mnz.x, mnz.y, mnz.z, mnz.w}, amxx[4] = {mxx.x, mxx.y, mxx.z, mxx.w},
                       amxy[4] = {mxy.x, mxy.y, mxy.z, mxy.w}, amxz[4] = {mxz.x, mxz.y, mxz.z, mxz.w};
@@ -399,6 +432,7 @@
           for (int i = 0; i < 4; i++)
             hit[i] = __builtin_amdgcn_ballot_w64(slab(amnx[i], amny[i], amnz[i], amxx[i], amxy[i], amxz[i], ox, oy, oz, ix, iy, iz, tm));
         }
+        IZPI_MARK("node_tail");
         const uint64_t m_inner = __builtin_amdgcn_ballot_w64(cur >= -1);
         const uint64_t b0 = hit[0] & __builtin_amdgcn_ballot_w64(ch.x != -1),
                        b1 = hit[1] & m_inner & __builtin_amdgcn_ballot_w64(ch.y != -1),
@@ -411,8 +445,12 @@
         const bool enter = ref_is_leaf(next) && (is_leaf || sc.leaf_shortcut);
         leaf_next = enter && !is_leaf;
         in_prim = enter;
-        pk = enter ? leaf_start(next) : pk;
-        pend = enter ? leaf_start(next) + leaf_count(next) : pend;
+        if constexpr (DIST) {
+          lref = enter ? next : lref;
+        } else {
+          pk = enter ? leaf_start(next) : pk;
+          pend = enter ? leaf_start(next) + leaf_count(next) : pend;
+        }
         next = enter ? -1 : next;
         const uint64_t r1 = b0 & b1, r2 = (b0 | b1) & b2, r3 = (b0 | b1 | b2) & b3;
         const int np_ = (int)lane_of(r1) + (int)lane_of(r2) + (int)lane_of(r3);
@@ -436,7 +474,13 @@
       const bool do_fin = advance && next == -1 && sp == 0;
       const int spn = sp - 1;
       int32_t top = *(volatile __attribute__((address_space(3))) int32_t*)&lds_stack[threadIdx.x + (spn & (S - 1)) * 256];
+#ifdef IZPI_TRACE_ICOUNT
+      if (__ballot(do_pop) != 0) ic_pop++;
+      if (__ballot(do_fin) != 0) ic_finish++;
+#endif
       if (any_spill && __ballot(do_pop && spn < low) != 0) {
+        IZPI_MARK("readback");
+        IZPI_IC(ic_readback);
         if (do_pop && spn < low) {
           top = gsp[(size_t)spn * spill_stride];
           low = spn;
@@ -446,15 +490,21 @@
         }
         __builtin_amdgcn_s_waitcnt(0x0F70);
       }
+      IZPI_MARK("advance_tail");
       cur = (advance && next != -1) ? next : (do_pop ? top : cur);
       sp = (advance && next == -1) ? spn : sp;
       const bool lf = do_pop && ref_is_leaf(top) && spn >= clean_from && sc.leaf_shortcut;
       in_prim = in_prim || lf;
       leaf_next = leaf_next || lf;
-      pk = lf ? leaf_start(top) : pk;
-      pend = lf ? leaf_start(top) + leaf_count(top) : pend;
+      if constexpr (DIST) {
+        lref = lf ? top : lref;
+      } else {
+        pk = lf ? leaf_start(top) : pk;
+        pend = lf ? leaf_start(top) + leaf_count(top) : pend;
+      }
       clean_from = (do_pop && spn < clean_from) ? spn : clean_from;
       if (do_fin) {
+        IZPI_MARK("finish");
         const double2 uv = (UVL && bprim >= 0) ? lds_uv[threadIdx.x] : make_double2(0.0, 0.0);
         if ((UVL || UVS) && wp.hit_uv) {
           double2* rec = wp.in.hit + ((size_t)qi << 1);
@@ -466,7 +516,8 @@
         busy = false;
       }
     }
-    const uint64_t n_short = (uint64_t)__popcll(__ballot(leaf_next));
+    IZPI_MARK("advance_end");
+    const uint64_t n_short = (uint64_t)__popcll(__builtin_amdgcn_ballot_w64(leaf_next));
     c_nodes += n_short;
     c_short += n_short;
 #ifdef IZPI_TRACE_CLOCKS
@@ -486,6 +537,20 @@
     if (c_spill_st) atomicAdd(counters + CNT_CLK_REFILL, (unsigned long long)c_spill_st);
     if (c_spill_ld) atomicAdd(counters + CNT_CLK_NODE, (unsigned long long)c_spill_ld);
     if (sh_acc == 0x9E3779B9u) atomicOr(err, 0u);
+  }
+#endif
+#ifdef IZPI_TRACE_ICOUNT
+  if (lane == 0) {
+    count_add(wp.cpart, counters, CNT_IC_ITER, ic_iter);
+    count_add(wp.cpart, counters, CNT_IC_IDLE, ic_idle);
+    count_add(wp.cpart, counters, CNT_IC_DEQUEUE, ic_dequeue);
+    count_add(wp.cpart, counters, CNT_IC_REFILL, ic_refill);
+    count_add(wp.cpart, counters, CNT_IC_TWIN, ic_twin);
+    count_add(wp.cpart, counters, CNT_IC_SPILL, ic_spill);
+    count_add(wp.cpart, counters, CNT_IC_READBACK, ic_readback);
+    count_add(wp.cpart, counters, CNT_IC_POP, ic_pop);
+    count_add(wp.cpart, counters, CNT_IC_FINISH, ic_finish);
+    count_add(wp.cpart, counters, CNT_IC_WAVES, 1);
   }
 #endif
   if (lane == 0) {
@@ -506,6 +571,7 @@
   X(true, true, false, true, false) X(true, false, true, true, false) X(true, true, true, true, false)               \
   X(true, false, false, false, true) X(true, true, false, false, true) X(true, true, false, true, true)
 constexpr int ring_of(bool lb, bool rl) { return lb && rl ? 8 : TRACE_RING; }
+int trace_ring(const Tracer& t) { return ring_of(t.lds_bvh, t.ray_lds); }
 
 int make_tracer(izpi_ctx* ctx, const izpi_render_tuning& tu, bool need_uv, Tracer* t) {
   *t = Tracer();
@@ -521,6 +587,7 @@
   t->ray_lds = t->p2 && ((t->tri && !t->lds_bvh && !need_uv) || (t->lds_bvh && (t->tri || ctx->sc.time_free))) &&
                !(tu.flags & IZPI_TUNE_NO_RAY_LDS);
   t->qnodes = ctx->sc.quantized && t->p2 && !t->lds_bvh && !(tu.flags & IZPI_TUNE_NO_QNODES);
+  t->a32 = ctx->sc.addr32 != 0 && !(tu.flags & IZPI_TUNE_WIDE_ADDR);
   if (tu.prim_weight) t->prim_w = tu.prim_weight;
   if (tu.trace_chunk) t->tchunk = tu.trace_chunk;
   if (tu.refill_min) t->refill_min = std::min<uint32_t>(64, tu.refill_min);
@@ -528,7 +595,8 @@
   ctx->err = "no k_trace2 instance for this scene and tuning";
 #define IZPI_T2_OCC(P, T, L, R, Q)                                                               \
   if (t->p2 == P && t->tri == T && t->lds_bvh == L && t->ray_lds == R && t->qnodes == Q) \
-    rc = resident_blocks(ctx, k_trace2<ring_of(L, R), TRACE_WPE, P, T, L, R, Q>, &t->blocks);
+    rc = t->a32 ? resident_blocks(ctx, k_trace2<ring_of(L, R), TRACE_WPE, P, T, L, R, Q, !L>, &t->blocks)       \
+                : resident_blocks(ctx, k_trace2<ring_of(L, R), TRACE_WPE, P, T, L, R, Q, false>, &t->blocks);
   IZPI_T2_LIST(IZPI_T2_OCC)
 #undef IZPI_T2_OCC
   if (rc) return rc;
@@ -541,8 +609,12 @@
   const uint32_t stride = (uint32_t)t.blocks * 256;
 #define IZPI_T2_LAUNCH(P, T, L, R, Q)                                                                          \
   if (t.p2 == P && t.tri == T && t.lds_bvh == L && t.ray_lds == R && t.qnodes == Q) {                          \
-    hipLaunchKernelGGL((k_trace2<ring_of(L, R), TRACE_WPE, P, T, L, R, Q>), g, b, 0, st, sc, wp, ctx->d_counters, \
-                       misc(ctx, 1), spill, stride, t.prim_w, t.tchunk, t.refill_min);                        \
+    if (t.a32)                                                                                                 \
+      hipLaunchKernelGGL((k_trace2<ring_of(L, R), TRACE_WPE, P, T, L, R, Q, !L>), g, b, 0, st, sc, wp,           \
+                         ctx->d_counters, misc(ctx, 1), spill, stride, t.prim_w, t.tchunk, t.refill_min);       \
+    else                                                                                                       \
+      hipLaunchKernelGGL((k_trace2<ring_of(L, R), TRACE_WPE, P, T, L, R, Q, false>), g, b, 0, st, sc, wp,        \
+                         ctx->d_counters, misc(ctx, 1), spill, stride, t.prim_w, t.tchunk, t.refill_min);       \
     return;                                                                                                    \
   }
   IZPI_T2_LIST(IZPI_T2_LAUNCH)
```

Measured after the change: 2619, median of 6. 1.0% higher.
